# GiannisPikoulis/dsml-thesis

Hardware: AMD Instinct MI355X
Metric: DDIM denoise steps/sec (64×64×4 latent, 256² face) at 1/2/4/8 GPUs (higher is better)
Workload: dtype f32; 1 GPU; face_reenactment emotion-conditioned LDM (AffectNet config), DDIM-200 schedule, 16 samples/GPU, 64x64x4 latent, CFG off, eta 0, random-init weights; batch_per_gpu=16, global_batch=16, ddim_steps=200, hipgraph=True

## Files before the change

dsml_thesis_amd/csrc/igemm.hip:

```cpp
#include "ldmk_common.h"
#include "ldmk_split.h"
#include "ldmk_epilogue.h"
#include <stdlib.h>

#if defined(LDMK_IG_STAMPS) && (LDMK_IG_STAMPS == 1 || LDMK_IG_STAMPS == 3)
#define IG_T(i) do { const unsigned long long t_ = __builtin_amdgcn_s_memtime(); ig_acc[i] += t_ - ig_last; ig_last = t_; } while (0)
#elif defined(LDMK_IG_STAMPS)
#define IG_T(i) do { (void)ig_acc; (void)ig_last; } while (0)
#else
#define IG_T(i) do { } while (0)
#endif

namespace ldmk {

template <int TM, int TN, int LEAN>
__device__ __forceinline__ void ig_lean_epilogue(const ldmk_igemm_args& p, f32x16 (&acc)[TM][TN], const int rowbase, const int colbase, const int bz,
                                                 const int l31, const int half) {
  float* __restrict__ outp = p.out + (long long)bz * p.out_bstride;
  const float* __restrict__ resp = (LEAN == 2 || LEAN == 4) ? p.residual + (long long)bz * p.out_bstride : nullptr;
  const float alpha = p.alpha;
#pragma unroll
  for (int j = 0; j < TN; ++j) {
    const int col = colbase + j * 32 + l31;
    const float bv = p.bias ? p.bias[col] : 0.f;
// ... 1166 lines not shown
}

static int g_force_cfg = 0;
extern "C" void ldmk_igemm_force_config(int cfg) { g_force_cfg = cfg; }

extern "C" int ldmk_igemm_plan(const ldmk_igemm_args* args, int* tile_cfg, int* splitk) {
  if (!args || !tile_cfg || !splitk) return LDMK_EINVAL;
  ldmk::plan(*args, tile_cfg, splitk, args->splitk_ws ? args->splitk_ws_elems : 0);
  return LDMK_OK;
}

extern "C" long long ldmk_igemm_workspace_elems(const ldmk_igemm_args* args) {
  using namespace ldmk;
  LDMK_REQUIRE(args != nullptr, "ldmk_igemm_workspace_elems: null args");
  const ldmk_igemm_args& a = *args;
  LDMK_REQUIRE(a.M > 0 && a.N > 0 && a.K > 0, "ldmk_igemm_workspace_elems: empty problem M=%d N=%d K=%d", a.M, a.N, a.K);
  LDMK_REQUIRE(a.splitk >= 0 && a.splitk <= 64, "ldmk_igemm_workspace_elems: splitk=%d outside [0,64]", a.splitk);
  int cfg = a.tile_cfg, sk = a.splitk;
  if (sk == 0) {
    int c2 = 0;
    plan(a, &c2, &sk, 1LL << 50);
    if (cfg == 0) cfg = c2;
  }
  if (cfg > kNumCfg + kNumRCfg + kNumSCfg)
    return sk <= 1 || a.epi == LDMK_EPI_GEGLU ? 0 : (long long)(a.batch > 1 ? a.batch : 1) * sk * (long long)a.M * a.N;
  if (cfg > kNumCfg + kNumRCfg) {
    if (sk <= 1 || (a.epi == LDMK_EPI_GEGLU && !a.raw_slabs)) return 0;
    return (long long)sk * (long long)a.M * a.N;
  }
  if (cfg > kNumCfg || a.epi == LDMK_EPI_GEGLU || sk <= 1) return 0;
  return (long long)(a.batch > 1 ? a.batch : 1) * sk * (long long)a.M * a.N;
}

static int igemm_entry(const ldmk_igemm_args* args, void* stream, bool launch);
extern "C" int ldmk_igemm(const ldmk_igemm_args* args, void* stream) { return igemm_entry(args, stream, true); }
extern "C" int ldmk_igemm_check(const ldmk_igemm_args* args) { return igemm_entry(args, nullptr, false); }

static int igemm_entry(const ldmk_igemm_args* args, void* stream, bool launch) {
  LDMK_ENTER();
  using namespace ldmk;
  LDMK_REQUIRE(args != nullptr, "ldmk_igemm: null args");
  ldmk_igemm_args a = *args;
  LDMK_REQUIRE(a.M > 0 && a.N > 0 && a.K > 0, "ldmk_igemm: empty problem M=%d N=%d K=%d", a.M, a.N, a.K);
  LDMK_REQUIRE(a.c0 > 0 && a.c0 % 32 == 0 && a.c1 % 32 == 0, "ldmk_igemm: channel counts must be multiples of 32 (c0=%d c1=%d)", a.c0, a.c1);
  LDMK_REQUIRE((a.c1 == 0) == (a.a1 == nullptr), "ldmk_igemm: a1/c1 mismatch");
  const int taps = a.a_mode == LDMK_A_CONV3X3 ? 9 : 1;
  const int skip_k = a.skip_a0 ? a.skip_c0 + a.skip_c1 : 0;
  LDMK_REQUIRE(a.K == taps * (a.c0 + a.c1) + skip_k, "ldmk_igemm: K=%d != taps*(c0+c1)+skip=%d", a.K, taps * (a.c0 + a.c1) + skip_k);
  LDMK_REQUIRE(!a.skip_a0 || (a.a_mode == LDMK_A_CONV3X3 && a.skip_c0 > 0 && a.skip_c0 % 8 == 0 && a.skip_c1 % 8 == 0 &&
                              (a.skip_c1 == 0) == (a.skip_a1 == nullptr) && (a.tile_cfg > kNumCfg + kNumRCfg || a.tile_cfg == 0)),
               "ldmk_igemm: the fused skip connection needs a 3x3 convolution on a slab-GEMM tile, skip channels in multiples of 8");
  LDMK_REQUIRE(a.N % 4 == 0 && a.ldb % 4 == 0, "ldmk_igemm: N and ldb must be multiples of 4");
  LDMK_REQUIRE(a.rows_per_sample > 0, "ldmk_igemm: rows_per_sample");
  LDMK_REQUIRE((long long)a.M * a.ldc < (1LL << 31) && a.ldc > 0, "ldmk_igemm: output exceeds 2^31 elements per batch item (32-bit epilogue offsets)");
  const long long samples = ((long long)a.M + a.rows_per_sample - 1) / a.rows_per_sample;
  if (a.a_mode == LDMK_A_CONV3X3) {
    LDMK_REQUIRE(a.in_h > 0 && a.in_w > 0 && a.out_h > 0 && a.out_w > 0 && a.stride >= 1, "ldmk_igemm: conv geometry");
    LDMK_REQUIRE(a.rows_per_sample == a.out_h * a.out_w, "ldmk_igemm: rows_per_sample != out_h*out_w");
    LDMK_REQUIRE(a.batch <= 1, "ldmk_igemm: batched conv unsupported");
    LDMK_REQUIRE(samples * a.in_h * a.in_w * (a.c0 > a.c1 ? a.c0 : a.c1) < (1LL << 31),
                 "ldmk_igemm: conv input exceeds 2^31 elements (32-bit gather indices)");
  } else {
    LDMK_REQUIRE((long long)a.M * (a.c0 > a.c1 ? a.c0 : a.c1) < (1LL << 31), "ldmk_igemm: A exceeds 2^31 elements per batch item");
  }
  if (a.a_tf == LDMK_TF_AFFINE || a.a_tf == LDMK_TF_AFFINE_SILU) LDMK_REQUIRE(a.tf_coef, "ldmk_igemm: tf_coef missing");
  if (a.a_tf == LDMK_TF_LAYERNORM) {
    LDMK_REQUIRE(a.row_stats && a.ln_gamma && a.ln_beta && a.a_mode == LDMK_A_ROWS, "ldmk_igemm: layernorm prologue args");
  }
  if (a.a_tf == LDMK_TF_LAYERNORM_FOLDED)
    LDMK_REQUIRE(a.row_stats && a.ln_colsum && a.a_mode == LDMK_A_ROWS && !a.stats_out && a.batch <= 1,
                 "ldmk_igemm: folded layernorm needs row_stats, ln_colsum (ldmk_fold_layernorm), rows mode, no stats_out, no batching");
  LDMK_REQUIRE(a.a_tf >= LDMK_TF_NONE && a.a_tf <= LDMK_TF_LAYERNORM_FOLDED, "ldmk_igemm: a_tf=%d", a.a_tf);
  if (a.epi == LDMK_EPI_GEGLU) LDMK_REQUIRE(a.N % 64 == 0 && !a.residual && !a.batch_vec, "ldmk_igemm: GEGLU needs N%%64==0 and no residual");
  if (a.stats_out)
    LDMK_REQUIRE(a.M % 32 == 0 && a.rows_per_sample % 32 == 0 && a.epi == LDMK_EPI_NONE && a.batch <= 1,
                 "ldmk_igemm: stats_out needs M%%32==0, rows_per_sample%%32==0, no GEGLU, no batching");
  LDMK_REQUIRE(a.tile_cfg >= 0 && a.tile_cfg <= kNumCfg + kNumRCfg + kNumSCfg + kNumWCfg + kNumPCfg, "ldmk_igemm: tile_cfg=%d outside [0,%d]",
               a.tile_cfg, kNumCfg + kNumRCfg + kNumSCfg + kNumWCfg + kNumPCfg);
  LDMK_REQUIRE(a.splitk >= 0 && a.splitk <= 64, "ldmk_igemm: splitk=%d outside [0,64]", a.splitk);
  LDMK_REQUIRE(a.compute == LDMK_COMPUTE_F32 || a.compute == LDMK_COMPUTE_BF16 || a.compute == LDMK_COMPUTE_BF16X3 || a.compute == LDMK_COMPUTE_F16X2,
               "ldmk_igemm: compute=%d", a.compute);
  const bool ps_tile = a.tile_cfg > kNumCfg + kNumRCfg + kNumSCfg + kNumWCfg;
  LDMK_REQUIRE(!a.a_ps1 || (ps_tile && a.a_ps), "ldmk_igemm: a_ps1 (second A source) is read by the pre-split tiles only, next to a_ps");
  if (a.compute == LDMK_COMPUTE_BF16X3 && !ps_tile) {
    LDMK_REQUIRE(a.w_split && !a.b_trans && a.w_split_ld >= a.K && a.w_split_ld % 8 == 0,
                 "ldmk_igemm: LDMK_COMPUTE_BF16X3 needs w_split (ldmk_pack_wsplit), b_trans = 0, w_split_ld >= K and a multiple of 8");
    LDMK_REQUIRE(3LL * a.N * a.w_split_ld * 2 < (1LL << 32), "ldmk_igemm: w_split exceeds 4 GB per batch entry");
    LDMK_REQUIRE(igemm_fast_gather_ok(a), "ldmk_igemm: LDMK_COMPUTE_BF16X3 needs the fast gather (no zero-insertion, two-source "
                 "upsampling or operands beyond 4 GB)");
  }
  if (a.compute == LDMK_COMPUTE_F16X2) {
    LDMK_REQUIRE(a.tile_cfg <= kNumCfg || ps_tile, "ldmk_igemm: LDMK_COMPUTE_F16X2 runs on the LDS-tiled shapes (tile_cfg 0..6) and the pre-split "
                 "tiles (23..28, 31..33), not tile_cfg=%d", a.tile_cfg);
    LDMK_REQUIRE(!a.a_split && a.w_scale_exp >= -60 && a.w_scale_exp <= 60, "ldmk_igemm: LDMK_COMPUTE_F16X2: a_split is not taken; w_scale_exp=%d", a.w_scale_exp);
    if (!ps_tile) {
      LDMK_REQUIRE(a.w_split && !a.b_trans && a.w_split_ld >= a.K && a.w_split_ld % 8 == 0 && 2LL * a.N * a.w_split_ld * 2 < (1LL << 32),
                   "ldmk_igemm: LDMK_COMPUTE_F16X2 needs w_split (ldmk_pack_wsplit_h2), b_trans = 0, w_split_ld >= K and a multiple of 8, below 4 GB");
      LDMK_REQUIRE(a.range_flag != nullptr, "ldmk_igemm: LDMK_COMPUTE_F16X2 needs range_flag");
      LDMK_REQUIRE(igemm_fast_gather_ok(a), "ldmk_igemm: LDMK_COMPUTE_F16X2 needs the fast gather (no zero-insertion, two-source upsampling or "
                   "operands beyond 4 GB)");
    }
  }
  if (a.compute == LDMK_COMPUTE_BF16 && a.w_split)
    LDMK_REQUIRE(!a.b_trans && a.w_split_ld >= a.K && a.w_split_ld % 8 == 0 && (long long)a.N * a.w_split_ld * 2 < (1LL << 32) && a.batch <= 1,
                 "ldmk_igemm: LDMK_COMPUTE_BF16 with w_split (ldmk_pack_wbf16t) needs b_trans = 0, w_split_ld >= K and a multiple of 8, "
                 "no batching");
  if (a.a_split) {
    LDMK_REQUIRE(a.compute == LDMK_COMPUTE_BF16X3 && a.a_mode == LDMK_A_ROWS && a.c1 == 0 && a.batch <= 1 &&
                 (a.a_tf == LDMK_TF_NONE || a.a_tf == LDMK_TF_LAYERNORM_FOLDED) && a.tile_cfg <= kNumCfg,
                 "ldmk_igemm: a_split (pre-split A) needs LDMK_COMPUTE_BF16X3 on an LDS-tiled shape (tile_cfg 0..6), rows mode, one "
                 "source, no staging prologue, no batching");
    LDMK_REQUIRE(a.a_split_ld >= a.K && a.a_split_ld % 8 == 0 && 3LL * a.M * a.a_split_ld * 2 < (1LL << 32),
                 "ldmk_igemm: a_split_ld=%d must be >= K, a multiple of 8, and the three images below 4 GB", a.a_split_ld);
  }
  LDMK_REQUIRE(a.compute == LDMK_COMPUTE_F32 || a.tile_cfg <= kNumCfg || a.tile_cfg > kNumCfg + kNumRCfg + kNumSCfg,
               "ldmk_igemm: the row / slab GEMM tiles are fp32 only");
  if (a.alpha == 0.f) a.alpha = 1.f;
  if (a.compute == LDMK_COMPUTE_F16X2) a.alpha *= ldexpf(1.f, -(LDMK_F16X2_A_EXP + a.w_scale_exp));
  int cfg = 0, sk = 1;
  plan(a, &cfg, &sk, a.splitk_ws ? a.splitk_ws_elems : 0);
  if (a.tile_cfg > 0) cfg = a.tile_cfg;
  if (g_force_cfg > 0 && (g_force_cfg <= kNumCfg || !rgemm_unsupported(a, g_force_cfg - kNumCfg - 1))) cfg = g_force_cfg;
  LDMK_REQUIRE(!a.skip_a0 || cfg > kNumCfg + kNumRCfg, "ldmk_igemm: the fused skip connection runs on the slab GEMM only (tile_cfg 13..20)");
  if (cfg > kNumCfg + kNumRCfg + kNumSCfg + kNumWCfg) {
    const int pcfg = cfg - kNumCfg - kNumRCfg - kNumSCfg - kNumWCfg - 1;
    int psk = a.splitk > 0 ? a.splitk : 1;
    const char* why = igemm_ps_unsupported(a, pcfg, psk);
    LDMK_REQUIRE(why == nullptr, "ldmk_igemm: tile_cfg=%d splitk=%d (pre-split bf16x3 tile) cannot run this problem: %s", cfg, psk, why ? why : "");
    LDMK_REQUIRE(!a.raw_slabs || psk >= 2, "ldmk_igemm: raw_slabs needs a split-K plan");
    if (psk > 1) {
      const long long b = a.batch > 1 ? a.batch : 1;
      LDMK_REQUIRE_MEM(a.splitk_ws && b * psk * (long long)a.M * a.N <= a.splitk_ws_elems,
                       "ldmk_igemm: splitk=%d needs a workspace of %lld floats (ldmk_igemm_workspace_elems), %lld given", psk,
                       b * psk * (long long)a.M * a.N, a.splitk_ws ? a.splitk_ws_elems : 0LL);
    }
    if (!launch) return LDMK_OK;
    return igemm_ps_dispatch(a, pcfg, psk, a.splitk_ws, (hipStream_t)stream);
  }
  if (cfg > kNumCfg + kNumRCfg + kNumSCfg) {
    const int wcfg = cfg - kNumCfg - kNumRCfg - kNumSCfg - 1;
    int wsk = a.splitk > 0 ? a.splitk : 1;
    const char* why = igemm_ws_unsupported(a, wcfg, wsk);
    LDMK_REQUIRE(why == nullptr, "ldmk_igemm: tile_cfg=%d splitk=%d (warp-specialised bf16x3 tile) cannot run this problem: %s", cfg, wsk,
                 why ? why : "");
    LDMK_REQUIRE(!a.raw_slabs || wsk >= 2, "ldmk_igemm: raw_slabs needs a split-K plan");
    if (wsk > 1) {
      const long long b = a.batch > 1 ? a.batch : 1;
      LDMK_REQUIRE_MEM(a.splitk_ws && b * wsk * (long long)a.M * a.N <= a.splitk_ws_elems,
                       "ldmk_igemm: splitk=%d needs a workspace of %lld floats (ldmk_igemm_workspace_elems), %lld given", wsk,
                       b * wsk * (long long)a.M * a.N, a.splitk_ws ? a.splitk_ws_elems : 0LL);
    }
    if (!launch) return LDMK_OK;
    return igemm_ws_dispatch(a, wcfg, wsk, a.splitk_ws, (hipStream_t)stream);
  }
  if (cfg > kNumCfg + kNumRCfg) {
    const int scfg = cfg - kNumCfg - kNumRCfg - 1;
    int ssk = a.splitk > 0 ? a.splitk : 1;
    const char* why = sgemm_unsupported(a, scfg, ssk);
    LDMK_REQUIRE(why == nullptr, "ldmk_igemm: tile_cfg=%d splitk=%d (slab GEMM) cannot run this problem: %s", cfg, ssk, why ? why : "");
    if (ssk > 1)
      LDMK_REQUIRE_MEM(a.splitk_ws && ssk * (long long)a.M * a.N <= a.splitk_ws_elems,
                       "ldmk_igemm: splitk=%d needs a workspace of %lld floats (ldmk_igemm_workspace_elems), %lld given", ssk,
                       ssk * (long long)a.M * a.N, a.splitk_ws ? a.splitk_ws_elems : 0LL);
    if (!launch) return LDMK_OK;
    return sgemm_dispatch(a, scfg, ssk, a.splitk_ws, (hipStream_t)stream);
  }
// ... 28 lines not shown
```

dsml_thesis_amd/csrc/igemm_ps.hip:

```cpp
#include "ldmk_common.h"
#include "ldmk_split.h"
#include "ldmk_epilogue.h"
#include <stdlib.h>

namespace ldmk {

#ifdef LDMK_PS_PROBES
constexpr bool PS_PROBES = true;
#else
constexpr bool PS_PROBES = false;
#endif
static int ps_probe_bits() {
  if (!PS_PROBES) return 0;
  static const int dbg = [] {
    const char* d = getenv("LDMK_PS_DEBUG");
    const char* s = getenv("LDMK_PS_STAGGER");
    return (d ? atoi(d) : 0) | ((s ? atoi(s) : 0) << 8);
  }();
  return dbg;
}

constexpr unsigned PS_OOB = 0x80000000u;

__device__ __forceinline__ void ps_dma3(unsigned voff, const u32x4& rs, unsigned lds_dst) {
  unsigned keep;
  asm volatile("s_nop 4\n\ts_mov_b32 %0, m0\n\ts_mov_b32 m0, %3\n\ts_nop 0\n\t"
               "buffer_load_dwordx4 %1, %2, 0 offen lds\n\t"
               "buffer_load_dwordx4 %1, %2, 0 offen offset:1024 lds\n\t"
               "buffer_load_dwordx4 %1, %2, 0 offen offset:2048 lds\n\t"
               "s_mov_b32 m0, %0"
               : "=&s"(keep) : "v"(voff), "s"(rs), "s"(lds_dst) : "memory");
}

template <int PL>
__device__ __forceinline__ void ps_dma(unsigned voff, const u32x4& rs, unsigned lds_dst) {
  if constexpr (PL == 3) {
    ps_dma3(voff, rs, lds_dst);
  } else {
    unsigned keep;
    asm volatile("s_nop 4\n\ts_mov_b32 %0, m0\n\ts_mov_b32 m0, %3\n\ts_nop 0\n\t"
                 "buffer_load_dwordx4 %1, %2, 0 offen lds\n\t"
                 "buffer_load_dwordx4 %1, %2, 0 offen offset:1024 lds\n\t"
                 "s_mov_b32 m0, %0"
                 : "=&s"(keep) : "v"(voff), "s"(rs), "s"(lds_dst) : "memory");
  }
}

__device__ __attribute__((aligned(16))) const float kPsZeros[4] = {0.f, 0.f, 0.f, 0.f};

constexpr int PS_KV_TILE = 16 * 1024;
template <int TM, int TN, bool TR, int PL = 3, bool KV = false, int LEAN = 0>
__device__ __forceinline__ void ps_epilogue(const ldmk_igemm_args& p, f32x16 (&acc)[TM][TN], const int rowbase, const int colbase,
                                            const int splitk, const int ks, const int bz, float* __restrict__ ws, const int lane,
                                            float* __restrict__ kv_ts = nullptr) {
  const int l31 = lane & 31, half = lane >> 5;
  const float alpha = p.alpha;
  constexpr bool L_ANY = LEAN != 0, L_LNF = LEAN == 1, L_RS = LEAN == 2 || LEAN == 4, L_BV = LEAN == 4;
  const bool lnf = L_ANY ? L_LNF : p.a_tf == LDMK_TF_LAYERNORM_FOLDED;
  const float2* __restrict__ stats2 = reinterpret_cast<const float2*>(p.row_stats);

  if constexpr (TR) {
    if (splitk > 1) {
      float* slab = ws + ((long long)bz * splitk + ks) * p.M * p.N;
#pragma unroll
      for (int i = 0; i < TM; ++i) {
        const int row = rowbase + 32 * i + l31;
        if (row >= p.M) continue;
#pragma unroll
        for (int j = 0; j < TN; ++j)
#pragma unroll
          for (int q = 0; q < 4; ++q) {
            const int col = colbase + 32 * j + 8 * q + 4 * half;
            if (col < p.N)
              *reinterpret_cast<float4*>(slab + (long long)row * p.N + col) =
                  make_float4(acc[i][j][4 * q], acc[i][j][4 * q + 1], acc[i][j][4 * q + 2], acc[i][j][4 * q + 3]);
          }
      }
      return;
    }
    float* __restrict__ outp = p.out ? p.out + (long long)bz * p.out_bstride : nullptr;
    unsigned char* __restrict__ ops_ = reinterpret_cast<unsigned char*>(p.out_ps);
    const bool geglu = p.epi == LDMK_EPI_GEGLU;
    const int Kbo = p.ldc / 16;
    const float* __restrict__ csp = lnf ? p.ln_colsum : kPsZeros;
    const float* __restrict__ bip = p.bias ? p.bias : kPsZeros;
    const float* __restrict__ rsp = p.residual ? p.residual + (long long)bz * p.out_bstride : kPsZeros;
    const unsigned mcs = lnf ? ~0u : 0u, mbi = p.bias ? ~0u : 0u, mrs = p.residual ? ~0u : 0u, mbv = p.batch_vec ? ~0u : 0u;
    bool bad_ps = false;
#pragma unroll
    for (int i = 0; i < TM; ++i) {
      const int row = rowbase + 32 * i + l31;
      const bool rok = L_ANY || row < p.M;
      const int rr = rok ? row : p.M - 1;
      float mean = 0.f, rstd = 1.f;
      if (lnf) { const float2 st = stats2[rr]; mean = st.x; rstd = st.y; }
      const float* __restrict__ bvp = p.batch_vec ? p.batch_vec + (long long)(rr / p.rows_per_sample) * p.batch_vec_ld : kPsZeros;
      const unsigned rowoff = (unsigned)rr * (unsigned)p.ldc;
      const long long psrow = ((long long)((rowbase + 32 * i) >> 5) * Kbo) * (PL * 1024) + l31 * 16 + half * 8;
      constexpr int JS = (TN % 2 == 0) ? 2 : 1;
#pragma unroll
      for (int j = 0; j < TN; j += JS) {
#pragma unroll
        for (int jj = 0; jj < JS; ++jj) {
          if (geglu && jj == 1) break;
          const int jt = j + jj;
          const int ctile = colbase + 32 * jt;
          if (!L_ANY && ctile >= p.N) continue;
          const int otile = geglu ? (ctile >> 1) : ctile;
          float kvv[KV ? 16 : 1];
          const bool kv_tile = KV && ctile >= p.N / 3;
#pragma unroll
          for (int qh = 0; qh < 4; qh += 2) {
          float4 cs[4], bi[4], bv[4], rs[4], csg[4], big[4];
#pragma unroll
          for (int q = qh; q < qh + 2; ++q) {
            const unsigned c = (unsigned)(ctile + 8 * q + 4 * half), oc = (unsigned)(otile + 8 * q + 4 * half);
            if constexpr (!L_ANY || L_LNF) cs[q] = *reinterpret_cast<const float4*>(csp + (c & mcs));
            bi[q] = *reinterpret_cast<const float4*>(bip + (c & mbi));
            if constexpr (!L_ANY) {
              bv[q] = *reinterpret_cast<const float4*>(bvp + (oc & mbv));
              rs[q] = *reinterpret_cast<const float4*>(rsp + ((rowoff + oc) & mrs));
            } else {
              if constexpr (L_RS) rs[q] = *reinterpret_cast<const float4*>(rsp + (rowoff + oc));
              if constexpr (L_BV) bv[q] = *reinterpret_cast<const float4*>(bvp + oc);
            }
            if constexpr (TN % 2 == 0) {
              if (geglu) {
                if constexpr (!L_ANY || L_LNF) csg[q] = *reinterpret_cast<const float4*>(csp + ((c + 32) & mcs));
                big[q] = *reinterpret_cast<const float4*>(bip + ((c + 32) & mbi));
              }
            }
          }
#pragma unroll
          for (int q = qh; q < qh + 2; ++q) {
            float4 v = make_float4(acc[i][jt][4 * q] * alpha, acc[i][jt][4 * q + 1] * alpha, acc[i][jt][4 * q + 2] * alpha,
                                   acc[i][jt][4 * q + 3] * alpha);
            if constexpr (L_LNF) {
              v.x = lnf_bias(v.x, mean, cs[q].x, rstd, bi[q].x); v.y = lnf_bias(v.y, mean, cs[q].y, rstd, bi[q].y);
              v.z = lnf_bias(v.z, mean, cs[q].z, rstd, bi[q].z); v.w = lnf_bias(v.w, mean, cs[q].w, rstd, bi[q].w);
            } else if constexpr (L_ANY) {
            } else {
              if (lnf) {
                v.x = fmaf(-mean, cs[q].x, v.x) * rstd; v.y = fmaf(-mean, cs[q].y, v.y) * rstd;
                v.z = fmaf(-mean, cs[q].z, v.z) * rstd; v.w = fmaf(-mean, cs[q].w, v.w) * rstd;
              }
              v.x += bi[q].x; v.y += bi[q].y; v.z += bi[q].z; v.w += bi[q].w;
            }
            if constexpr (TN % 2 == 0) {
              if (geglu) {
                constexpr int TNm1 = TN - 1;
                const int jg = jt + 1 < TN ? jt + 1 : TNm1;
                float4 g = make_float4(acc[i][jg][4 * q] * alpha, acc[i][jg][4 * q + 1] * alpha, acc[i][jg][4 * q + 2] * alpha,
                                       acc[i][jg][4 * q + 3] * alpha);
                if constexpr (L_LNF) {
                  g.x = lnf_bias(g.x, mean, csg[q].x, rstd, big[q].x); g.y = lnf_bias(g.y, mean, csg[q].y, rstd, big[q].y);
                  g.z = lnf_bias(g.z, mean, csg[q].z, rstd, big[q].z); g.w = lnf_bias(g.w, mean, csg[q].w, rstd, big[q].w);
                } else {
                  if (lnf) {
                    g.x = fmaf(-mean, csg[q].x, g.x) * rstd; g.y = fmaf(-mean, csg[q].y, g.y) * rstd;
                    g.z = fmaf(-mean, csg[q].z, g.z) * rstd; g.w = fmaf(-mean, csg[q].w, g.w) * rstd;
                  }
                  g.x += big[q].x; g.y += big[q].y; g.z += big[q].z; g.w += big[q].w;
                }
                v.x *= gelu_erf_f(g.x); v.y *= gelu_erf_f(g.y); v.z *= gelu_erf_f(g.z); v.w *= gelu_erf_f(g.w);
              }
            }
            if constexpr (L_LNF) {
              v.x += 0.f; v.y += 0.f; v.z += 0.f; v.w += 0.f;
            } else if constexpr (L_ANY) {
              const float4 r4 = L_RS ? rs[q] : make_float4(0.f, 0.f, 0.f, 0.f), b4 = L_BV ? bv[q] : make_float4(0.f, 0.f, 0.f, 0.f);
              v.x = bias_res(v.x, bi[q].x, b4.x, r4.x); v.y = bias_res(v.y, bi[q].y, b4.y, r4.y);
              v.z = bias_res(v.z, bi[q].z, b4.z, r4.z); v.w = bias_res(v.w, bi[q].w, b4.w, r4.w);
            } else {
              v.x += bv[q].x; v.y += bv[q].y; v.z += bv[q].z; v.w += bv[q].w;
              v.x += rs[q].x; v.y += rs[q].y; v.z += rs[q].z; v.w += rs[q].w;
            }
            if constexpr (KV) {
              if (kv_tile) { kvv[4 * q] = v.x; kvv[4 * q + 1] = v.y; kvv[4 * q + 2] = v.z; kvv[4 * q + 3] = v.w; }
            }
            if (rok && !kv_tile) {
              const int oc = otile + 8 * q + 4 * half;
              if (outp) *reinterpret_cast<float4*>(outp + rowoff + oc) = v;
              if (ops_) {
                unsigned char* d = ops_ + psrow + (long long)((otile >> 4) + (q >> 1)) * (PL * 1024) + (q & 1) * 512;
                if constexpr (PL == 3) {
                  bf16x4 h, m, l;
                  split3(v, h, m, l);
                  *reinterpret_cast<bf16x4*>(d) = h;
                  *reinterpret_cast<bf16x4*>(d + 1024) = m;
                  *reinterpret_cast<bf16x4*>(d + 2048) = l;
                } else {
                  bad_ps |= h2_out_of_range(v);
                  f16x4 h, l;
                  split2h(scaled_sat(v), h, l);
                  *reinterpret_cast<f16x4*>(d) = h;
                  *reinterpret_cast<f16x4*>(d + 1024) = l;
                }
              }
            }
          }
          }
          if constexpr (KV) {
            if (kv_tile && (L_ANY || rowbase + 32 * i < p.M)) {
              const int Cq = p.N / 3;
              const int sec = ctile / Cq;
              const int hh = (ctile - sec * Cq) >> 5;
              const int r0 = rowbase + 32 * i;
              const int bsm = r0 / p.attn_tokens, key0 = r0 - bsm * p.attn_tokens;
              const int ntl = p.attn_tokens >> 6;
              unsigned char* dst = reinterpret_cast<unsigned char*>(p.attn_kv_out) +
                                   (((long long)bsm * (Cq >> 5) + hh) * ntl + (key0 >> 6)) * PS_KV_TILE + lane * 16;
              const int sub = (key0 >> 5) & 1;
              bool bad = false;
              if (sec == 1) {
#pragma unroll
                for (int t = 0; t < 2; ++t) {
                  float vals[8];
#pragma unroll
                  for (int e = 0; e < 4; ++e) {
                    const auto r = __builtin_amdgcn_permlane32_swap(__float_as_uint(kvv[8 * t + e]), __float_as_uint(kvv[8 * t + 4 + e]), false, false);
                    vals[e] = __uint_as_float(r[0]);
                    vals[4 + e] = __uint_as_float(r[1]);
                  }
                  const float4 v0 = make_float4(vals[0], vals[1], vals[2], vals[3]), v1 = make_float4(vals[4], vals[5], vals[6], vals[7]);
                  bad |= h2_out_of_range(v0) || h2_out_of_range(v1);
                  f16x4 h0, l0, h1, l1;
                  split2h(scaled_sat(v0), h0, l0);
                  split2h(scaled_sat(v1), h1, l1);
                  unsigned char* d = dst + (2 * sub + t) * 2048;
                  *reinterpret_cast<f16x8*>(d) = f16x8{h0[0], h0[1], h0[2], h0[3], h1[0], h1[1], h1[2], h1[3]};
                  *reinterpret_cast<f16x8*>(d + 1024) = f16x8{l0[0], l0[1], l0[2], l0[3], l1[0], l1[1], l1[2], l1[3]};
                }
              } else {
#pragma unroll
                for (int q = 0; q < 4; ++q)
#pragma unroll
                  for (int e = 0; e < 4; ++e) kv_ts[l31 * 33 + 8 * q + 4 * half + e] = kvv[4 * q + e];
                __builtin_amdgcn_s_waitcnt(0xC07F);
                __builtin_amdgcn_wave_barrier();
#pragma unroll
                for (int t = 0; t < 2; ++t) {
                  float vals[8];
#pragma unroll
                  for (int jx = 0; jx < 8; ++jx) vals[jx] = kv_ts[(16 * t + 4 * half + (jx & 3) + 8 * (jx >> 2)) * 33 + l31];
                  const float4 v0 = make_float4(vals[0], vals[1], vals[2], vals[3]), v1 = make_float4(vals[4], vals[5], vals[6], vals[7]);
                  bad |= h2_out_of_range(v0) || h2_out_of_range(v1);
                  f16x4 h0, l0, h1, l1;
                  split2h(scaled_sat(v0), h0, l0);
                  split2h(scaled_sat(v1), h1, l1);
                  unsigned char* d = dst + (4 + 2 * sub + t) * 2048;
                  *reinterpret_cast<f16x8*>(d) = f16x8{h0[0], h0[1], h0[2], h0[3], h1[0], h1[1], h1[2], h1[3]};
                  *reinterpret_cast<f16x8*>(d + 1024) = f16x8{l0[0], l0[1], l0[2], l0[3], l1[0], l1[1], l1[2], l1[3]};
                }
                __builtin_amdgcn_s_waitcnt(0xC07F);
                __builtin_amdgcn_wave_barrier();
              }
              if (bad) *p.range_flag = 1;
            }
          }
        }
      }
    }
    if (bad_ps) *p.range_flag = 1;
    return;
  } else {
    if (splitk > 1) {
      col_slab_store<TM, TN>(p, acc, rowbase, colbase, bz, l31, half, splitk, ks, ws);
      return;
    }
    if (p.epi == LDMK_EPI_GEGLU) {
      col_geglu<TM, TN>(p, acc, rowbase, colbase, bz, l31, half, lnf);
      return;
    }
    if constexpr (LEAN != 0) col_lean<TM, TN, LEAN>(p, acc, rowbase, colbase, bz, l31, half);
    else col_general<TM, TN>(p, acc, rowbase, colbase, bz, l31, half, lnf);
  }
}

template <bool TR>
__device__ __forceinline__ int ps_lean_form(const ldmk_igemm_args& p, const int splitk, const bool off, const int row_end, const int col_end) {
  if constexpr (!TR) {
    return col_lean_form(p, splitk, off, row_end, col_end);
  } else {
    if (off || splitk != 1 || row_end > p.M || col_end > p.N) return 0;
    if (p.batch_vec && p.rows_per_sample % 32 != 0) return 0;
    if (p.a_tf == LDMK_TF_LAYERNORM_FOLDED) return p.residual || p.batch_vec ? 0 : 1;
    if (p.epi == LDMK_EPI_GEGLU || (p.batch_vec && !p.residual)) return 0;
    return p.batch_vec ? 4 : (p.residual ? 2 : 3);
  }
}

template <int NWM, int NWN, int TM, int TN, int NS, bool TR, int PL = 3, bool KV = false>
__global__ __launch_bounds__(64 * NWM * NWN, 2) void igemm_ps_kernel(const ldmk_igemm_args p, const int splitk, float* __restrict__ ws, const int dbg_arg, const int nfast) {
  const int dbg = PS_PROBES ? dbg_arg : 0;
  constexpr int NW = NWM * NWN;
  constexpr int BM = 32 * TM * NWM, BN = 32 * TN * NWN;
  constexpr int FA = BM / 32, FB = BN / 32, U = FA + FB;
  constexpr int UHI = (U + NW - 1) / NW, ULO = U / NW;
  constexpr int UB = PL * 1024;
  constexpr int STAGE = U * UB;
  static_assert(PL * UHI * (NS - 1) <= 63, "vmcnt is a 6-bit counter");
  extern __shared__ __attribute__((aligned(1024))) unsigned char smem_ps[];

  const int tid = threadIdx.x, lane = tid & 63, wave = __builtin_amdgcn_readfirstlane(tid >> 6);
  const int l31 = lane & 31, half = lane >> 5;
  const int wm = wave / NWN, wn = wave - wm * NWN;

  const int tiles_m = (p.M + BM - 1) / BM;
  const int tiles_n = (p.N + BN - 1) / BN;
  const int bid = xcd_remap(blockIdx.x, tiles_m * tiles_n);
  const int m0 = (nfast & 1) ? (bid / tiles_n) * BM : (bid % tiles_m) * BM;
  const int n0 = (nfast & 1) ? (bid % tiles_n) * BN : (bid / tiles_m) * BN;
  const int ks = blockIdx.y, bz = blockIdx.z;

  const int nkc = p.K / 32;
  const int it_per = (nkc + splitk - 1) / splitk;
  const int it_begin = ks * it_per;
  const int it_end = min(nkc, it_begin + it_per);
  const int n16 = it_end > it_begin ? 2 * (it_end - it_begin) : 0;
  const int Kb = p.K / 16;
  const int Mb = (p.M + 31) / 32, Nb = p.N / 32;

  const int Ka0 = p.a_ps1 ? p.a_ps_k0 / 16 : Kb, Ka1 = Kb - Ka0;
  const u32x4 rs_a = buffer_rsrc(reinterpret_cast<const unsigned char*>(p.a_ps) + (long long)bz * p.a_ps_bstride, (dbg & 1) ? 0u : (unsigned)Mb * (unsigned)Ka0 * (unsigned)UB);
  const u32x4 rs_a1 = buffer_rsrc(p.a_ps1 ? p.a_ps1 : p.a_ps, (dbg & 1) ? 0u : (unsigned)Mb * (unsigned)Ka1 * (unsigned)UB);
  const u32x4 rs_b = buffer_rsrc(reinterpret_cast<const unsigned char*>(p.w_ps) + (long long)bz * p.w_ps_bstride, (dbg & 1) ? 0u : (unsigned)Nb * (unsigned)Kb * (unsigned)UB);
  unsigned ubase[UHI], ubase1[UHI];
#pragma unroll
  for (int i = 0; i < UHI; ++i) {
    const int u = wave + NW * i;
    const int blk = u < FA ? m0 / 32 + u : n0 / 32 + (u - FA);
    const bool ok = u < U && (u < FA ? blk < Mb : blk < Nb);
    ubase[i] = ok ? (unsigned)blk * (unsigned)(u < FA ? Ka0 : Kb) * (unsigned)UB + (unsigned)(2 * it_begin) * (unsigned)UB : PS_OOB;
    ubase1[i] = (unsigned)blk * (unsigned)Ka1 * (unsigned)UB + (unsigned)(2 * it_begin - Ka0) * (unsigned)UB;
  }
  const unsigned lane16 = lane * 16;
  const unsigned lds0 = (unsigned)(size_t)smem_ps;
  auto issue = [&](int s) {
    const unsigned buf = lds0 + (unsigned)(s % NS) * STAGE;
    const bool live = s < n16;
    const bool src1 = 2 * it_begin + s >= Ka0;
    const u32x4 rs_as = src1 ? rs_a1 : rs_a;
#pragma unroll
    for (int i = 0; i < UHI; ++i) {
      const int u = wave + NW * i;
      if (u < U && !(dbg & 2)) {
        const unsigned off = (live && ubase[i] != PS_OOB) ? ((u < FA && src1) ? ubase1[i] : ubase[i]) + (unsigned)s * (unsigned)UB : PS_OOB;
        ps_dma<PL>(lane16 + off, u < FA ? rs_as : rs_b, buf + (unsigned)u * (unsigned)UB);
      }
    }
  };
  const bool hi_wave = wave + NW * (UHI - 1) < U;

  f32x16 acc[TM][TN];
#pragma unroll
  for (int i = 0; i < TM; ++i)
#pragma unroll
    for (int j = 0; j < TN; ++j)
#pragma unroll
      for (int r = 0; r < 16; ++r) acc[i][j][r] = 0.f;

  if ((dbg >> 8) != 0) {
    const unsigned slot = __builtin_amdgcn_s_getreg(6148);
    if (slot & 1) {
      const int n = (dbg >> 8) * n16;
      for (int i = 0; i < n; i += 64) __builtin_amdgcn_s_sleep(64);
    }
  }
#pragma unroll
  for (int s = 0; s < NS - 1; ++s) issue(s);
  for (int it = 0; it < n16; ++it) {
    if (hi_wave) wait_vm<PL * UHI * (NS - 2)>(); else wait_vm<PL * ULO * (NS - 2)>();
    asm volatile("s_barrier" ::: "memory");
    issue(it + NS - 1);
    const unsigned char* sb = smem_ps + (it % NS) * STAGE + lane16;
    bf16x8 a8[PL][TM];
#pragma unroll
    for (int g = 0; g < PL; ++g)
#pragma unroll
      for (int i = 0; i < TM; ++i) a8[g][i] = *reinterpret_cast<const bf16x8*>(sb + ((wm * TM + i) * PL + g) * 1024);
#pragma unroll
    for (int j = 0; j < TN; ++j) {
      bf16x8 b8[PL];
#pragma unroll
      for (int g = 0; g < PL; ++g) b8[g] = *reinterpret_cast<const bf16x8*>(sb + ((FA + wn * TN + j) * PL + g) * 1024);
      if (dbg & 4) {
#pragma unroll
        for (int i = 0; i < TM; ++i)
#pragma unroll
          for (int g = 0; g < PL; ++g) asm volatile("" :: "v"(a8[g][i]), "v"(b8[g]));
        continue;
      }
#pragma unroll
      for (int i = 0; i < TM; ++i) {
        if constexpr (PL == 2) {
          const f16x8 ah = __builtin_bit_cast(f16x8, a8[0][i]), al = __builtin_bit_cast(f16x8, a8[1][i]);
          const f16x8 bh = __builtin_bit_cast(f16x8, b8[0]), bl = __builtin_bit_cast(f16x8, b8[1]);
          if constexpr (TR) {
            acc[i][j] = __builtin_amdgcn_mfma_f32_32x32x16_f16(bh, al, acc[i][j], 0, 0, 0);
            acc[i][j] = __builtin_amdgcn_mfma_f32_32x32x16_f16(bl, ah, acc[i][j], 0, 0, 0);
            acc[i][j] = __builtin_amdgcn_mfma_f32_32x32x16_f16(bh, ah, acc[i][j], 0, 0, 0);
          } else {
            acc[i][j] = __builtin_amdgcn_mfma_f32_32x32x16_f16(al, bh, acc[i][j], 0, 0, 0);
            acc[i][j] = __builtin_amdgcn_mfma_f32_32x32x16_f16(ah, bl, acc[i][j], 0, 0, 0);
            acc[i][j] = __builtin_amdgcn_mfma_f32_32x32x16_f16(ah, bh, acc[i][j], 0, 0, 0);
          }
        } else if constexpr (TR) {
          acc[i][j] = __builtin_amdgcn_mfma_f32_32x32x16_bf16(b8[0], a8[2][i], acc[i][j], 0, 0, 0);
          acc[i][j] = __builtin_amdgcn_mfma_f32_32x32x16_bf16(b8[2], a8[0][i], acc[i][j], 0, 0, 0);
          acc[i][j] = __builtin_amdgcn_mfma_f32_32x32x16_bf16(b8[1], a8[1][i], acc[i][j], 0, 0, 0);
          acc[i][j] = __builtin_amdgcn_mfma_f32_32x32x16_bf16(b8[0], a8[1][i], acc[i][j], 0, 0, 0);
          acc[i][j] = __builtin_amdgcn_mfma_f32_32x32x16_bf16(b8[1], a8[0][i], acc[i][j], 0, 0, 0);
          acc[i][j] = __builtin_amdgcn_mfma_f32_32x32x16_bf16(b8[0], a8[0][i], acc[i][j], 0, 0, 0);
        } else {
          acc[i][j] = __builtin_amdgcn_mfma_f32_32x32x16_bf16(a8[2][i], b8[0], acc[i][j], 0, 0, 0);
          acc[i][j] = __builtin_amdgcn_mfma_f32_32x32x16_bf16(a8[0][i], b8[2], acc[i][j], 0, 0, 0);
          acc[i][j] = __builtin_amdgcn_mfma_f32_32x32x16_bf16(a8[1][i], b8[1], acc[i][j], 0, 0, 0);
          acc[i][j] = __builtin_amdgcn_mfma_f32_32x32x16_bf16(a8[1][i], b8[0], acc[i][j], 0, 0, 0);
          acc[i][j] = __builtin_amdgcn_mfma_f32_32x32x16_bf16(a8[0][i], b8[1], acc[i][j], 0, 0, 0);
          acc[i][j] = __builtin_amdgcn_mfma_f32_32x32x16_bf16(a8[0][i], b8[0], acc[i][j], 0, 0, 0);
        }
      }
    }
  }
  wait_vm<0>();
  if (dbg & 16) {
    float keep = 0.f;
#pragma unroll
    for (int i = 0; i < TM; ++i)
#pragma unroll
      for (int j = 0; j < TN; ++j)
#pragma unroll
        for (int r = 0; r < 16; ++r) keep += acc[i][j][r];
    if (keep == 12345.678f && ws) ws[0] = keep;
    return;
  }
  const int lean = ps_lean_form<TR>(p, splitk, (nfast & 2) != 0, m0 + (wm + 1) * 32 * TM, n0 + (wn + 1) * 32 * TN);
  if constexpr (KV) {
    __syncthreads();
    if (lean == 1)
      ps_epilogue<TM, TN, TR, PL, true, TR ? 1 : 0>(p, acc, m0 + wm * 32 * TM, n0 + wn * 32 * TN, splitk, ks, bz, ws, lane,
                                                    reinterpret_cast<float*>(smem_ps) + wave * (32 * 33));
    else
      ps_epilogue<TM, TN, TR, PL, true>(p, acc, m0 + wm * 32 * TM, n0 + wn * 32 * TN, splitk, ks, bz, ws, lane,
                                         reinterpret_cast<float*>(smem_ps) + wave * (32 * 33));
  } else {
    if (lean == 1) ps_epilogue<TM, TN, TR, PL, false, 1>(p, acc, m0 + wm * 32 * TM, n0 + wn * 32 * TN, splitk, ks, bz, ws, lane);
    else if (lean == 2) ps_epilogue<TM, TN, TR, PL, false, 2>(p, acc, m0 + wm * 32 * TM, n0 + wn * 32 * TN, splitk, ks, bz, ws, lane);
    else if (lean == 3) ps_epilogue<TM, TN, TR, PL, false, 3>(p, acc, m0 + wm * 32 * TM, n0 + wn * 32 * TN, splitk, ks, bz, ws, lane);
    else if (lean == 4) ps_epilogue<TM, TN, TR, PL, false, 4>(p, acc, m0 + wm * 32 * TM, n0 + wn * 32 * TN, splitk, ks, bz, ws, lane);
    else ps_epilogue<TM, TN, TR, PL>(p, acc, m0 + wm * 32 * TM, n0 + wn * 32 * TN, splitk, ks, bz, ws, lane);
  }
}

template <int TM, int TN, int NS, bool TR>
__global__ __launch_bounds__(512) void igemm_pw_kernel(const ldmk_igemm_args p, const int splitk, float* __restrict__ ws, const int dbg_arg) {
  const int dbg = PS_PROBES ? dbg_arg : 0;
  constexpr int BM = 128 * TM, BN = 32 * TN;
  constexpr int FA = BM / 32, FB = TN, U = FA + FB;
  constexpr int UHI = (U + 3) / 4, ULO = U / 4;
  constexpr int STAGE = U * 3072;
  static_assert(NS >= 3 && 3 * UHI * (NS - 2) <= 63, "ring depth / vmcnt range");
  extern __shared__ __attribute__((aligned(1024))) unsigned char smem_ps[];

  const int tid = threadIdx.x, lane = tid & 63, wave = __builtin_amdgcn_readfirstlane(tid >> 6);
  const int tiles_m = (p.M + BM - 1) / BM;
  const int tiles_n = (p.N + BN - 1) / BN;
  const int bid = xcd_remap(blockIdx.x, tiles_m * tiles_n);
  const int m0 = (bid % tiles_m) * BM;
  const int n0 = (bid / tiles_m) * BN;
  const int ks = blockIdx.y, bz = blockIdx.z;
  const int nkc = p.K / 32;
  const int it_per = (nkc + splitk - 1) / splitk;
  const int it_begin = ks * it_per;
  const int it_end = min(nkc, it_begin + it_per);
  const int n16 = it_end > it_begin ? 2 * (it_end - it_begin) : 0;
  const unsigned lane16 = lane * 16;

  if (wave >= 4) {
    const int pw = wave - 4;
    const int Kb = p.K / 16;
    const int Mb = (p.M + 31) / 32, Nb = p.N / 32;
    const u32x4 rs_a = buffer_rsrc(reinterpret_cast<const unsigned char*>(p.a_ps) + (long long)bz * p.a_ps_bstride, (dbg & 1) ? 0u : (unsigned)Mb * (unsigned)Kb * 3072u);
    const u32x4 rs_b = buffer_rsrc(reinterpret_cast<const unsigned char*>(p.w_ps) + (long long)bz * p.w_ps_bstride, (dbg & 1) ? 0u : (unsigned)Nb * (unsigned)Kb * 3072u);
    unsigned ubase[UHI];
#pragma unroll
    for (int i = 0; i < UHI; ++i) {
      const int u = pw + 4 * i;
      const int blk = u < FA ? m0 / 32 + u : n0 / 32 + (u - FA);
      const bool ok = u < U && (u < FA ? blk < Mb : blk < Nb);
      ubase[i] = ok ? (unsigned)blk * (unsigned)Kb * 3072u + (unsigned)(2 * it_begin) * 3072u : PS_OOB;
    }
    const unsigned lds0 = (unsigned)(size_t)smem_ps;
    auto issue = [&](int s) {
      const unsigned buf = lds0 + (unsigned)(s % NS) * STAGE;
      const bool live = s < n16;
#pragma unroll
      for (int i = 0; i < UHI; ++i) {
        const int u = pw + 4 * i;
        if (u < U && !(dbg & 2)) {
          const unsigned off = (live && ubase[i] != PS_OOB) ? ubase[i] + (unsigned)s * 3072u : PS_OOB;
          ps_dma3(lane16 + off, u < FA ? rs_a : rs_b, buf + (unsigned)u * 3072u);
        }
      }
    };
    const bool hi_wave = pw + 4 * (UHI - 1) < U;
    unsigned long long t_acc[3] = {0, 0, 0}, t_last = __builtin_amdgcn_s_memtime();
    const unsigned long long t_begin = t_last;
#define PW_T(i) do { if (dbg & 8) { const unsigned long long t_ = __builtin_amdgcn_s_memtime(); t_acc[i] += t_ - t_last; t_last = t_; } } while (0)
#pragma unroll
    for (int s = 0; s < NS - 1; ++s) issue(s);
    PW_T(0);
    if (hi_wave) wait_vm<3 * UHI * (NS - 2)>(); else wait_vm<3 * ULO * (NS - 2)>();
    PW_T(1);
    asm volatile("s_barrier" ::: "memory");
    PW_T(2);
    for (int it = 0; it < n16; ++it) {
      if (hi_wave) wait_vm<3 * UHI * (NS - 3)>(); else wait_vm<3 * ULO * (NS - 3)>();
      PW_T(1);
      asm volatile("s_barrier" ::: "memory");
      PW_T(2);
      issue(it + NS - 1);
      PW_T(0);
    }
    wait_vm<0>();
    if ((dbg & 8) && lane == 0 && p.splitk_counters) {
      unsigned long long* d = reinterpret_cast<unsigned long long*>(p.splitk_counters) + ((long long)blockIdx.x * 8 + wave) * 4;
      d[0] = t_acc[0]; d[1] = t_acc[1]; d[2] = t_acc[2]; d[3] = __builtin_amdgcn_s_memtime() - t_begin;
    }
    return;
// ... 120 lines not shown
    split3(make_float4(v[0], v[1], v[2], v[3]), h0, m0, l0);
    split3(make_float4(v[4], v[5], v[6], v[7]), h1, m1, l1);
    *reinterpret_cast<bf16x8*>(d) = bf16x8{h0[0], h0[1], h0[2], h0[3], h1[0], h1[1], h1[2], h1[3]};
    *reinterpret_cast<bf16x8*>(d + 1024) = bf16x8{m0[0], m0[1], m0[2], m0[3], m1[0], m1[1], m1[2], m1[3]};
    *reinterpret_cast<bf16x8*>(d + 2048) = bf16x8{l0[0], l0[1], l0[2], l0[3], l1[0], l1[1], l1[2], l1[3]};
  }
}

template <int KCH, int PL = 3>
__global__ __launch_bounds__(256) void ln_stats_ps_kernel(const float* __restrict__ x, int rows, int K, float eps, float* __restrict__ stats,
                                                          unsigned char* __restrict__ dst, float guard, int* __restrict__ flag,
                                                          int* __restrict__ range_flag) {
  const int rb = blockIdx.x;
  const int r = threadIdx.x >> 3, o = threadIdx.x & 7;
  const int row = rb * 32 + r;
  const bool rok = row < rows;
  const float* px = x + (long long)(rok ? row : 0) * K;
  float4 v[KCH][2];
  float s = 0.f;
#pragma unroll
  for (int c = 0; c < KCH; ++c) {
    const int k0 = c * 64 + o * 8;
    if (rok && k0 < K) {
      v[c][0] = *reinterpret_cast<const float4*>(px + k0);
      v[c][1] = *reinterpret_cast<const float4*>(px + k0 + 4);
    } else {
      v[c][0] = v[c][1] = make_float4(0.f, 0.f, 0.f, 0.f);
    }
    s += ((v[c][0].x + v[c][0].y) + (v[c][0].z + v[c][0].w)) + ((v[c][1].x + v[c][1].y) + (v[c][1].z + v[c][1].w));
  }
#pragma unroll
  for (int d = 4; d > 0; d >>= 1) s += __shfl_xor(s, d, 64);
  const float mean = s / (float)K;
  float q = 0.f;
#pragma unroll
  for (int c = 0; c < KCH; ++c) {
    if (c * 64 + o * 8 < K) {
#pragma unroll
      for (int e = 0; e < 2; ++e) {
        const float a = v[c][e].x - mean, b = v[c][e].y - mean, cc = v[c][e].z - mean, d = v[c][e].w - mean;
        q = fmaf(a, a, q); q = fmaf(b, b, q); q = fmaf(cc, cc, q); q = fmaf(d, d, q);
      }
    }
  }
#pragma unroll
  for (int d = 4; d > 0; d >>= 1) q += __shfl_xor(q, d, 64);
  if (rok && o == 0) {
    const float rstd = 1.0f / sqrtf(q / (float)K + eps);
    stats[2 * (long long)row] = mean;
    stats[2 * (long long)row + 1] = rstd;
    if (flag && !(fabsf(mean) * rstd <= guard)) *flag = 1;
  }
#pragma unroll
  for (int c = 0; c < KCH; ++c) {
    const int k0 = c * 64 + o * 8;
    if (k0 < K) {
      unsigned char* d = dst + ((long long)rb * (K / 16) + (k0 >> 4)) * (PL * 1024) + ((o & 1) * 32 + r) * 16;
      if constexpr (PL == 2) {
        if (h2_out_of_range(v[c][0]) || h2_out_of_range(v[c][1])) *range_flag = 1;
        f16x4 h0, l0, h1, l1;
        split2h(scaled_sat(v[c][0]), h0, l0);
        split2h(scaled_sat(v[c][1]), h1, l1);
        *reinterpret_cast<f16x8*>(d) = f16x8{h0[0], h0[1], h0[2], h0[3], h1[0], h1[1], h1[2], h1[3]};
        *reinterpret_cast<f16x8*>(d + 1024) = f16x8{l0[0], l0[1], l0[2], l0[3], l1[0], l1[1], l1[2], l1[3]};
      } else {
        bf16x4 h0, m0, l0, h1, m1, l1;
        split3(v[c][0], h0, m0, l0);
        split3(v[c][1], h1, m1, l1);
        *reinterpret_cast<bf16x8*>(d) = bf16x8{h0[0], h0[1], h0[2], h0[3], h1[0], h1[1], h1[2], h1[3]};
        *reinterpret_cast<bf16x8*>(d + 1024) = bf16x8{m0[0], m0[1], m0[2], m0[3], m1[0], m1[1], m1[2], m1[3]};
        *reinterpret_cast<bf16x8*>(d + 2048) = bf16x8{l0[0], l0[1], l0[2], l0[3], l1[0], l1[1], l1[2], l1[3]};
      }
    }
  }
}

int launch_splitk_reduce(const ldmk_igemm_args& a, int splitk, float* ws, hipStream_t st);

struct PsCfg { int bm, bn; bool even_tn; };
static const PsCfg kPsCfg[] = {{256, 160, false}, {256, 320, false}, {256, 256, true}, {128, 320, false}, {128, 160, false}, {128, 256, true},
                               {256, 160, false}, {256, 128, true},
                               {256, 160, false}, {256, 128, true}, {128, 256, true}};

template <int NWM, int NWN, int TM, int TN, int NS, bool TR, int PL = 3, bool KV = false>
static int ps_launch(const ldmk_igemm_args& a, int splitk, float* ws, hipStream_t st) {
  constexpr int BM = 32 * TM * NWM, BN = 32 * TN * NWN;
  constexpr size_t lds = (size_t)NS * (BM / 32 + BN / 32) * PL * 1024;
  static_assert(lds <= 160 * 1024, "LDS ring exceeds 160 KiB");
  static bool attr = false;
  if (!attr) {
    (void)hipFuncSetAttribute(reinterpret_cast<const void*>(igemm_ps_kernel<NWM, NWN, TM, TN, NS, TR, PL, KV>),
                              hipFuncAttributeMaxDynamicSharedMemorySize, (int)lds);
    attr = true;
  }
  const int tiles = ((a.M + BM - 1) / BM) * ((a.N + BN - 1) / BN);
  const int dbg = ps_probe_bits();
  static_assert(!KV || (size_t)NWM * NWN * 32 * 33 * 4 <= lds, "V^T transpose scratch fits the ring");
  const int nfast_env = switch_value(SW_PS_NFAST);
  const int lean_env = switch_value(SW_PS_LEAN);
  const int nfast = (nfast_env && (a.N + BN - 1) / BN > 1 && (a.M + BM - 1) / BM >= 8 ? 1 : 0) | (lean_env ? 0 : 2);
  hipLaunchKernelGGL((igemm_ps_kernel<NWM, NWN, TM, TN, NS, TR, PL, KV>), dim3(tiles, splitk, a.batch > 1 ? a.batch : 1), dim3(64 * NWM * NWN), lds,
                     st, a, splitk, ws, dbg, nfast);
  if (splitk > 1 && !a.raw_slabs) return launch_splitk_reduce(a, splitk, ws, st);
  return check_launch("ldmk_igemm(ps)");
}

template <int TM, int TN, int NS, bool TR>
static int pw_launch(const ldmk_igemm_args& a, int splitk, float* ws, hipStream_t st) {
  constexpr int BM = 128 * TM, BN = 32 * TN;
  constexpr size_t lds = (size_t)NS * (BM / 32 + TN) * 3072;
  static_assert(lds <= 160 * 1024, "LDS ring exceeds 160 KiB");
  static bool attr = false;
  if (!attr) {
    (void)hipFuncSetAttribute(reinterpret_cast<const void*>(igemm_pw_kernel<TM, TN, NS, TR>), hipFuncAttributeMaxDynamicSharedMemorySize, (int)lds);
    attr = true;
  }
  const int tiles = ((a.M + BM - 1) / BM) * ((a.N + BN - 1) / BN);
  const int dbg = ps_probe_bits() & 0xff;
  hipLaunchKernelGGL((igemm_pw_kernel<TM, TN, NS, TR>), dim3(tiles, splitk, a.batch > 1 ? a.batch : 1), dim3(512), lds, st, a, splitk, ws, dbg);
  if (splitk > 1 && !a.raw_slabs) return launch_splitk_reduce(a, splitk, ws, st);
  return check_launch("ldmk_igemm(pw)");
}

template <int NWM, int NWN, int TM, int TN, bool TR>
__global__ __launch_bounds__(64 * NWM * NWN, 2) void igemm_psc_kernel(const ldmk_igemm_args p, const int splitk, float* __restrict__ ws, const int nfast) {
  constexpr int PL = 2, NS = 3;
  constexpr int NW = NWM * NWN;
  constexpr int BM = 32 * TM * NWM, BN = 32 * TN * NWN;
  constexpr int FA = BM / 32, FB = BN / 32, U = FA + FB;
  constexpr int UHI = (U + NW - 1) / NW, ULO = U / NW;
  constexpr int AI = (FA + NW - 1) / NW;
  constexpr int UB = PL * 1024;
  constexpr int STAGE = U * UB;
  static_assert(18 % NS == 0 && PL * UHI * (NS - 1) <= 63, "ring / vmcnt");
  extern __shared__ __attribute__((aligned(1024))) unsigned char smem_ps[];

  const int tid = threadIdx.x, lane = tid & 63, wave = __builtin_amdgcn_readfirstlane(tid >> 6);
  const int l31 = lane & 31, half = lane >> 5;
  const int wm = wave / NWN, wn = wave - wm * NWN;
  const int tiles_m = (p.M + BM - 1) / BM;
  const int tiles_n = (p.N + BN - 1) / BN;
  const int bid = xcd_remap(blockIdx.x, tiles_m * tiles_n);
  const int m0 = (nfast & 1) ? (bid / tiles_n) * BM : (bid % tiles_m) * BM;
  const int n0 = (nfast & 1) ? (bid % tiles_n) * BN : (bid / tiles_m) * BN;
  const int ks = blockIdx.y;

  const int C = p.c0;
  const int nc32 = C / 32;
  const int c_per = (nc32 + splitk - 1) / splitk;
  const int c_begin = ks * c_per;
  const int c_end = min(nc32, c_begin + c_per);
  const int Kb_in = C / 16, Kb_w = p.K / 16;
  const int Nb = p.N / 32;
  const long long samples = ((long long)p.M + p.rows_per_sample - 1) / p.rows_per_sample;
  const unsigned Mb_in = (unsigned)((samples * p.in_h * p.in_w + 31) / 32);
  const u32x4 rs_a = buffer_rsrc(p.a_ps, Mb_in * (unsigned)Kb_in * (unsigned)UB);
  const u32x4 rs_b = buffer_rsrc(p.w_ps, (unsigned)Nb * (unsigned)Kb_w * (unsigned)UB);

  unsigned toff[AI][9];
#pragma unroll
  for (int i = 0; i < AI; ++i) {
    const int u = wave + NW * i;
    const int row = m0 + 32 * u + l31;
    const bool rok = u < FA && row < p.M;
    const int rr = rok ? row : 0;
    const int n = rr / p.rows_per_sample, rem = rr - n * p.rows_per_sample;
    const int oy = rem / p.out_w, ox = rem - oy * p.out_w;
#pragma unroll
    for (int t = 0; t < 9; ++t) {
      const int iy = oy * p.stride + t / 3 - p.pad_lo, ix = ox * p.stride + t % 3 - p.pad_lo;
      const bool ok = rok && iy >= 0 && iy < p.in_h && ix >= 0 && ix < p.in_w;
      const unsigned q = (unsigned)((n * p.in_h + iy) * p.in_w + ix);
      toff[i][t] = ok ? (q >> 5) * (unsigned)Kb_in * (unsigned)UB + ((unsigned)half * 32u + (q & 31u)) * 16u : PS_OOB;
    }
  }
  unsigned ubase[UHI];
#pragma unroll
  for (int i = 0; i < UHI; ++i) {
    const int u = wave + NW * i;
    const int blk = n0 / 32 + (u - FA);
    ubase[i] = (u >= FA && u < U && blk < Nb) ? (unsigned)blk * (unsigned)Kb_w * (unsigned)UB + (unsigned)(18 * c_begin) * (unsigned)UB : PS_OOB;
  }
  const unsigned lane16 = lane * 16;
  const unsigned lds0 = (unsigned)(size_t)smem_ps;
// ... 80 lines not shown
  const int k0 = kc * 64 + o * 8;
  if (k0 >= C) return;
  float4 v0 = make_float4(0.f, 0.f, 0.f, 0.f), v1 = v0;
  if (row < rows) {
    const float* src = k0 < c0 ? x0 + row * c0 + k0 : x1 + row * c1 + (k0 - c0);
    const float4 a = *reinterpret_cast<const float4*>(src), b = *reinterpret_cast<const float4*>(src + 4);
    const float* cf = coef + ((row / hw) * 2) * C + k0;
    const float4 s0 = *reinterpret_cast<const float4*>(cf), s1 = *reinterpret_cast<const float4*>(cf + 4);
    const float4 h0 = *reinterpret_cast<const float4*>(cf + C), h1 = *reinterpret_cast<const float4*>(cf + C + 4);
    v0 = make_float4(fmaf(a.x, s0.x, h0.x), fmaf(a.y, s0.y, h0.y), fmaf(a.z, s0.z, h0.z), fmaf(a.w, s0.w, h0.w));
    v1 = make_float4(fmaf(b.x, s1.x, h1.x), fmaf(b.y, s1.y, h1.y), fmaf(b.z, s1.z, h1.z), fmaf(b.w, s1.w, h1.w));
    if (silu) {
      v0 = make_float4(silu_f(v0.x), silu_f(v0.y), silu_f(v0.z), silu_f(v0.w));
      v1 = make_float4(silu_f(v1.x), silu_f(v1.y), silu_f(v1.z), silu_f(v1.w));
    }
    if (h2_out_of_range(v0) || h2_out_of_range(v1)) *range_flag = 1;
  }
  unsigned char* d = dst + ((long long)rb * (C / 16) + (k0 >> 4)) * 2048 + ((o & 1) * 32 + r) * 16;
  f16x4 a0, l0, a1, l1;
  split2h(scaled_sat(v0), a0, l0);
  split2h(scaled_sat(v1), a1, l1);
  *reinterpret_cast<f16x8*>(d) = f16x8{a0[0], a0[1], a0[2], a0[3], a1[0], a1[1], a1[2], a1[3]};
  *reinterpret_cast<f16x8*>(d + 1024) = f16x8{l0[0], l0[1], l0[2], l0[3], l1[0], l1[1], l1[2], l1[3]};
}

template <int NWM, int NWN, int TM, int TN, bool TR>
static int psc_launch(const ldmk_igemm_args& a, int splitk, float* ws, hipStream_t st) {
  constexpr int BM = 32 * TM * NWM, BN = 32 * TN * NWN;
  constexpr size_t lds = (size_t)3 * (BM / 32 + BN / 32) * 2048;
  static_assert(lds <= 160 * 1024, "LDS ring exceeds 160 KiB");
  static bool attr = false;
  if (!attr) {
    (void)hipFuncSetAttribute(reinterpret_cast<const void*>(igemm_psc_kernel<NWM, NWN, TM, TN, TR>), hipFuncAttributeMaxDynamicSharedMemorySize, (int)lds);
    attr = true;
  }
  const int tiles = ((a.M + BM - 1) / BM) * ((a.N + BN - 1) / BN);
  const int nfast_env = switch_value(SW_PS_NFAST);
  const int lean_env = switch_value(SW_PS_LEAN);
  const int nfast = (nfast_env && (a.N + BN - 1) / BN > 1 && (a.M + BM - 1) / BM >= 8 ? 1 : 0) | (lean_env ? 0 : 2);
  hipLaunchKernelGGL((igemm_psc_kernel<NWM, NWN, TM, TN, TR>), dim3(tiles, splitk, 1), dim3(64 * NWM * NWN), lds, st, a, splitk, ws, nfast);
  if (splitk > 1 && !a.raw_slabs) return launch_splitk_reduce(a, splitk, ws, st);
  return check_launch("ldmk_igemm(ps, conv)");
}

const char* igemm_ps_unsupported(const ldmk_igemm_args& a, int pcfg, int splitk) {
  if (a.compute != LDMK_COMPUTE_BF16X3 && a.compute != LDMK_COMPUTE_F16X2) return "the pre-split tiles run the bf16x3 and the f16x2 arithmetic (compute)";
  const int pl = a.compute == LDMK_COMPUTE_F16X2 ? 2 : 3;
  if (pl == 2 && (pcfg == 6 || pcfg == 7)) return "the warp-specialised pre-split tiles (29 / 30) exist in the bf16x3 arithmetic only";
  if (pl == 2 && a.out_ps && !a.range_flag) return "out_ps in the f16x2 arithmetic needs range_flag";
  if (!a.a_ps || !a.w_ps) return "a_ps / w_ps (operands in the PS layout: ldmk_pack_ps, ldmk_ln_stats_ps, out_ps of a producer GEMM)";
  if (a.a_mode == LDMK_A_CONV3X3) {
    if (pl != 2) return "the conv-mode pre-split tile runs the f16x2 arithmetic only";
    if (pcfg != 0 && pcfg != 1 && pcfg != 3 && pcfg != 4) return "conv mode: tile_cfg 23 / 24 / 26 / 27";
    if (a.c1 || a.a1 || a.upsample || a.a_tf != LDMK_TF_NONE || a.out_ps || a.batch > 1 || a.epi != LDMK_EPI_NONE || a.attn_kv_out)
      return "conv mode: one pre-normalised source (ldmk_gn_apply_ps_h2), no upsampling / prologue / out_ps / batching / GEGLU";
    if (a.c0 % 32) return "conv mode: C_in must be a multiple of 32";
    if ((a.c0 / 32) % splitk) return "conv mode: splitk must divide C_in / 32 (K is split on 32-channel chunk boundaries)";
    const long long smp = ((long long)a.M + a.rows_per_sample - 1) / a.rows_per_sample;
    if (((smp * a.in_h * a.in_w + 31) / 32) * (a.c0 / 16) * 2048 >= (1LL << 31)) return "conv mode: input of 2 GiB or more";
  } else if (a.a_mode != LDMK_A_ROWS) {
    return "rows mode or 3x3 convolution";
  }
  if (a.b_trans || a.upsample || a.skip_a0 || (a.splitk_counters && !(ps_probe_bits() & 8))) return "b_trans / upsample / fused skip / in-launch combine";
  if (a.a_tf != LDMK_TF_NONE && a.a_tf != LDMK_TF_LAYERNORM_FOLDED) return "no staging prologue: a_ps is what gets multiplied";
  if (a.K % 32 || a.N % 32) return "K and N must be multiples of 32";
  if (a.a_ps1) {
    if (a.a_mode != LDMK_A_ROWS || pcfg == 6 || pcfg == 7) return "a_ps1: rows mode on tile_cfg 23..28 / 31..33 (not the conv-mode or warp-specialised tiles)";
    if (a.batch > 1 || a.attn_kv_out || a.a_tf != LDMK_TF_NONE || a.epi == LDMK_EPI_GEGLU)
      return "a_ps1: no batching, no fused QKV tiles, no folded LayerNorm, no GEGLU";
    if (a.a_ps_k0 <= 0 || a.a_ps_k0 >= a.K || a.a_ps_k0 % 32) return "a_ps1: a_ps_k0 and K - a_ps_k0 must be positive multiples of 32";
  }
  const long long kb = a.K / 16;
  if ((a.a_mode == LDMK_A_ROWS && (long long)((a.M + 31) / 32) * kb * pl * 1024 >= (1LL << 31)) || (long long)(a.N / 32) * kb * pl * 1024 >= (1LL << 31))
    return "an operand of 2 GiB or more";
  if (a.epi == LDMK_EPI_GEGLU && (!kPsCfg[pcfg].even_tn || splitk > 1)) return "GEGLU needs a tile of (value, gate) pairs (256x256, 128x256) and no split-K";
  if (splitk > a.K / 32) return "more K slices than 32-deep chunks";
  if (a.out_ps) {
    if (splitk > 1 || a.batch > 1 || a.stats_out) return "out_ps: no split-K, no batching, no GroupNorm records (transposed epilogue)";
    if (a.ldc % 16) return "out_ps: ldc (the PS output's column count) must be a multiple of 16";
  } else if (!a.out && splitk <= 1) {
    return "no output";
  }
  if (a.stats_out && !a.out) return "stats_out needs out";
  if (a.attn_kv_out) {
    if (pl != 2 || (pcfg != 0 && pcfg != 4)) return "attn_kv_out: the F16X2 arithmetic on tile_cfg 23 / 27";
    if (a.stats_out || splitk > 1 || a.batch > 1 || a.epi != LDMK_EPI_NONE || a.out_ps || !a.out || !a.range_flag)
      return "attn_kv_out: the fused QKV projection (no split-K / batching / GEGLU / records / out_ps; out and range_flag required)";
    if (a.attn_heads <= 0 || a.N != 3 * 32 * a.attn_heads) return "attn_kv_out: N must be 3 x 32 x attn_heads ([q | k | v] of d_head 32)";
    if (a.attn_tokens <= 0 || a.attn_tokens % 64 || a.M % a.attn_tokens) return "attn_kv_out: attn_tokens a multiple of 64 that divides M";
  }
  return nullptr;
}

int igemm_ps_dispatch(const ldmk_igemm_args& a, int pcfg, int splitk, float* ws, hipStream_t st) {
  const bool tr = !a.stats_out;
  if (a.a_mode == LDMK_A_CONV3X3) {
    switch (pcfg) {
      case 0: return tr ? psc_launch<8, 1, 1, 5, true>(a, splitk, ws, st) : psc_launch<8, 1, 1, 5, false>(a, splitk, ws, st);
      case 1: return tr ? psc_launch<4, 2, 2, 5, true>(a, splitk, ws, st) : psc_launch<4, 2, 2, 5, false>(a, splitk, ws, st);
      case 3: return tr ? psc_launch<4, 2, 1, 5, true>(a, splitk, ws, st) : psc_launch<4, 2, 1, 5, false>(a, splitk, ws, st);
      default: return tr ? psc_launch<4, 1, 1, 5, true>(a, splitk, ws, st) : psc_launch<4, 1, 1, 5, false>(a, splitk, ws, st);
    }
  }
  if (a.compute == LDMK_COMPUTE_F16X2 && a.attn_kv_out)
    return pcfg == 0 ? ps_launch<8, 1, 1, 5, 3, true, 2, true>(a, splitk, ws, st) : ps_launch<4, 1, 1, 5, 3, true, 2, true>(a, splitk, ws, st);
  if (a.compute == LDMK_COMPUTE_F16X2) {
    switch (pcfg) {
      case 0: return tr ? ps_launch<8, 1, 1, 5, 3, true, 2>(a, splitk, ws, st) : ps_launch<8, 1, 1, 5, 3, false, 2>(a, splitk, ws, st);
      case 1: return tr ? ps_launch<4, 2, 2, 5, 3, true, 2>(a, splitk, ws, st) : ps_launch<4, 2, 2, 5, 3, false, 2>(a, splitk, ws, st);
      case 2: return tr ? ps_launch<4, 2, 2, 4, 3, true, 2>(a, splitk, ws, st) : ps_launch<4, 2, 2, 4, 3, false, 2>(a, splitk, ws, st);
      case 3: return tr ? ps_launch<4, 2, 1, 5, 3, true, 2>(a, splitk, ws, st) : ps_launch<4, 2, 1, 5, 3, false, 2>(a, splitk, ws, st);
      case 4: return tr ? ps_launch<4, 1, 1, 5, 3, true, 2>(a, splitk, ws, st) : ps_launch<4, 1, 1, 5, 3, false, 2>(a, splitk, ws, st);
      case 8: return tr ? ps_launch<4, 1, 2, 5, 3, true, 2>(a, splitk, ws, st) : ps_launch<4, 1, 2, 5, 3, false, 2>(a, splitk, ws, st);
      case 9: return tr ? ps_launch<4, 1, 2, 4, 3, true, 2>(a, splitk, ws, st) : ps_launch<4, 1, 2, 4, 3, false, 2>(a, splitk, ws, st);
      case 10: return tr ? ps_launch<2, 2, 2, 4, 3, true, 2>(a, splitk, ws, st) : ps_launch<2, 2, 2, 4, 3, false, 2>(a, splitk, ws, st);
      default: return tr ? ps_launch<4, 2, 1, 4, 3, true, 2>(a, splitk, ws, st) : ps_launch<4, 2, 1, 4, 3, false, 2>(a, splitk, ws, st);
    }
  }
  switch (pcfg) {
    case 0: return tr ? ps_launch<8, 1, 1, 5, 3, true>(a, splitk, ws, st) : ps_launch<8, 1, 1, 5, 3, false>(a, splitk, ws, st);
    case 1: return tr ? ps_launch<4, 2, 2, 5, 2, true>(a, splitk, ws, st) : ps_launch<4, 2, 2, 5, 2, false>(a, splitk, ws, st);
    case 2: return tr ? ps_launch<4, 2, 2, 4, 3, true>(a, splitk, ws, st) : ps_launch<4, 2, 2, 4, 3, false>(a, splitk, ws, st);
    case 3: return tr ? ps_launch<4, 2, 1, 5, 3, true>(a, splitk, ws, st) : ps_launch<4, 2, 1, 5, 3, false>(a, splitk, ws, st);
    case 4: return tr ? ps_launch<4, 1, 1, 5, 2, true>(a, splitk, ws, st) : ps_launch<4, 1, 1, 5, 2, false>(a, splitk, ws, st);
    case 6: return tr ? pw_launch<2, 5, 4, true>(a, splitk, ws, st) : pw_launch<2, 5, 4, false>(a, splitk, ws, st);
    case 7: return tr ? pw_launch<2, 4, 4, true>(a, splitk, ws, st) : pw_launch<2, 4, 4, false>(a, splitk, ws, st);
    case 8: return tr ? ps_launch<4, 1, 2, 5, 2, true>(a, splitk, ws, st) : ps_launch<4, 1, 2, 5, 2, false>(a, splitk, ws, st);
    case 9: return tr ? ps_launch<4, 1, 2, 4, 2, true>(a, splitk, ws, st) : ps_launch<4, 1, 2, 4, 2, false>(a, splitk, ws, st);
    case 10: return tr ? ps_launch<2, 2, 2, 4, 2, true>(a, splitk, ws, st) : ps_launch<2, 2, 2, 4, 2, false>(a, splitk, ws, st);
    default: return tr ? ps_launch<4, 2, 1, 4, 3, true>(a, splitk, ws, st) : ps_launch<4, 2, 1, 4, 3, false>(a, splitk, ws, st);
  }
}

}

extern "C" long long ldmk_ps_bytes(int rows, int k) {
  if (rows <= 0 || k <= 0 || k % 16) return -1;
  return (long long)((rows + 31) / 32) * (k / 16) * 3072;
}

extern "C" long long ldmk_ps_bytes_h2(int rows, int k) {
  if (rows <= 0 || k <= 0 || k % 16) return -1;
  return (long long)((rows + 31) / 32) * (k / 16) * 2048;
}

extern "C" int ldmk_pack_ps(const float* src, int rows, int k, long long row_stride, long long k_stride, int batch, long long src_bstride,
                            void* dst, void* stream) {
  LDMK_ENTER();
  using namespace ldmk;
  LDMK_REQUIRE(src && dst && rows > 0 && k > 0 && batch >= 1, "ldmk_pack_ps: bad args");
  LDMK_REQUIRE(k % 16 == 0, "ldmk_pack_ps: k=%d must be a multiple of 16", k);
  LDMK_REQUIRE(k_stride != 1 || (row_stride % 4 == 0 && (reinterpret_cast<uintptr_t>(src) & 15) == 0 && src_bstride % 4 == 0),
               "ldmk_pack_ps: row-major sources are read as float4 (16-byte aligned rows)");
  const long long bytes = ldmk_ps_bytes(rows, k);
  hipLaunchKernelGGL(pack_ps_kernel<3>, dim3((rows + 31) / 32, (k + 63) / 64, batch), dim3(256), 0, (hipStream_t)stream, src, rows, k, row_stride,
                     k_stride, src_bstride, reinterpret_cast<unsigned char*>(dst), bytes, 1.0f, (int*)nullptr);
  return check_launch("ldmk_pack_ps");
}

extern "C" int ldmk_pack_ps_h2(const float* src, int rows, int k, long long row_stride, long long k_stride, int batch, long long src_bstride,
                               int scale_exp, int* range_flag, void* dst, void* stream) {
  LDMK_ENTER();
  using namespace ldmk;
  LDMK_REQUIRE(src && dst && rows > 0 && k > 0 && batch >= 1, "ldmk_pack_ps_h2: bad args");
  LDMK_REQUIRE(k % 16 == 0, "ldmk_pack_ps_h2: k=%d must be a multiple of 16", k);
  LDMK_REQUIRE(k_stride != 1 || (row_stride % 4 == 0 && (reinterpret_cast<uintptr_t>(src) & 15) == 0 && src_bstride % 4 == 0),
               "ldmk_pack_ps_h2: row-major sources are read as float4 (16-byte aligned rows)");
  LDMK_REQUIRE(scale_exp >= -60 && scale_exp <= 60, "ldmk_pack_ps_h2: scale_exp=%d outside [-60, 60]", scale_exp);
  LDMK_REQUIRE(!range_flag || scale_exp == LDMK_F16X2_A_EXP, "ldmk_pack_ps_h2: range_flag is the activations' check: scale_exp must be %d", LDMK_F16X2_A_EXP);
  const long long bytes = ldmk_ps_bytes_h2(rows, k);
  hipLaunchKernelGGL(pack_ps_kernel<2>, dim3((rows + 31) / 32, (k + 63) / 64, batch), dim3(256), 0, (hipStream_t)stream, src, rows, k, row_stride,
                     k_stride, src_bstride, reinterpret_cast<unsigned char*>(dst), bytes, ldexpf(1.f, scale_exp), range_flag);
  return check_launch("ldmk_pack_ps_h2");
}

extern "C" int ldmk_ln_stats_ps(const float* x, int rows, int c, float eps, float* stats, void* dst, float guard, int* flag, void* stream) {
  LDMK_ENTER();
  using namespace ldmk;
  LDMK_REQUIRE(x && stats && dst && rows > 0 && c > 0, "ldmk_ln_stats_ps: bad args");
  LDMK_REQUIRE(c % 16 == 0 && c <= 1280, "ldmk_ln_stats_ps: C=%d must be a multiple of 16, at most 1280", c);
  LDMK_REQUIRE(!flag || guard > 0.f, "ldmk_ln_stats_ps: guard=%g must be positive", (double)guard);
  const dim3 grid((rows + 31) / 32);
  unsigned char* d = reinterpret_cast<unsigned char*>(dst);
  hipStream_t st = (hipStream_t)stream;
// ... 39 lines not shown
```

dsml_thesis_amd/lib.py:

```python
import ctypes as C
import os

from . import switches

_HERE = os.path.dirname(os.path.abspath(__file__))
LIB_PATH = switches.get("LDMK_LIBRARY") or os.path.join(_HERE, "libldmk.so")

A_ROWS, A_CONV3X3 = 0, 1
TF_NONE, TF_AFFINE, TF_AFFINE_SILU, TF_LAYERNORM, TF_LAYERNORM_FOLDED = 0, 1, 2, 3, 4
EPI_NONE, EPI_GEGLU = 0, 1
COMPUTE_F32, COMPUTE_BF16, COMPUTE_BF16X3, COMPUTE_F16X2 = 0, 1, 2, 3
POST_NONE, POST_GROUPNORM, POST_LAYERNORM = 0, 1, 2
PLMS_MULTISTEP, PLMS_PREDICTOR, PLMS_CORRECTOR = 0, 1, 2

_fp = C.c_void_p


class IgemmArgs(C.Structure):
    _fields_ = [
        ("M", C.c_int), ("N", C.c_int), ("K", C.c_int),
        ("a0", _fp), ("a1", _fp), ("c0", C.c_int), ("c1", C.c_int),
        ("a_mode", C.c_int), ("in_h", C.c_int), ("in_w", C.c_int), ("out_h", C.c_int), ("out_w", C.c_int),
        ("stride", C.c_int), ("pad_lo", C.c_int), ("upsample", C.c_int),
        ("a_tf", C.c_int), ("tf_coef", _fp), ("row_stats", _fp), ("ln_gamma", _fp), ("ln_beta", _fp),
        ("rows_per_sample", C.c_int),
        ("w", _fp), ("b_trans", C.c_int), ("ldb", C.c_int),
        ("bias", _fp), ("batch_vec", _fp), ("batch_vec_ld", C.c_int),
        ("residual", _fp), ("epi", C.c_int),
        ("out", _fp), ("ldc", C.c_int), ("batch", C.c_int),
        ("a_bstride", C.c_longlong), ("w_bstride", C.c_longlong), ("out_bstride", C.c_longlong),
        ("alpha", C.c_float), ("tile_cfg", C.c_int), ("splitk", C.c_int),
        ("splitk_ws", _fp), ("splitk_ws_elems", C.c_longlong), ("stats_out", _fp), ("compute", C.c_int), ("splitk_counters", _fp), ("splitk_counters_len", C.c_int),
        ("w_frag", _fp),
        ("ln_colsum", _fp),
        ("raw_slabs", C.c_int),
        ("skip_a0", _fp), ("skip_a1", _fp), ("skip_c0", C.c_int), ("skip_c1", C.c_int),
        ("w_split", _fp), ("w_split_ld", C.c_int), ("w_split_bstride", C.c_longlong),
        ("a_split", _fp), ("a_split_ld", C.c_int),
        ("a_ps", _fp), ("a_ps_bstride", C.c_longlong), ("w_ps", _fp), ("w_ps_bstride", C.c_longlong), ("out_ps", _fp),
        ("w_scale_exp", C.c_int), ("range_flag", _fp),
        ("attn_kv_out", _fp), ("attn_tokens", C.c_int), ("attn_heads", C.c_int),
        ("a_ps1", _fp), ("a_ps_k0", C.c_int),
    ]


class PostArgs(C.Structure):
    _fields_ = [
        ("src", _fp), ("nslab", C.c_int), ("slab_stride", C.c_longlong), ("M", C.c_int), ("N", C.c_int),
        ("rows_per_sample", C.c_int), ("alpha", C.c_float), ("bias", _fp), ("batch_vec", _fp), ("batch_vec_ld", C.c_int),
        ("residual", _fp), ("ldr", C.c_int), ("geglu", C.c_int), ("raw_out", _fp), ("ld_raw", C.c_int), ("norm", C.c_int),
        ("x1", _fp), ("c1", C.c_int), ("groups", C.c_int), ("eps", C.c_float), ("gamma", _fp), ("beta", _fp),
        ("silu", C.c_int), ("norm_out", _fp), ("ld_norm", C.c_int), ("gn_cache_floats", C.c_int),
        ("gn_scratch", _fp), ("gn_scratch_elems", C.c_longlong),
    ]


class WgradArgs(C.Structure):
    _fields_ = [
        ("R", C.c_int), ("Kw", C.c_int), ("N", C.c_int), ("a", _fp), ("c", C.c_int), ("lda", C.c_int),
        ("a_mode", C.c_int), ("in_h", C.c_int), ("in_w", C.c_int), ("out_h", C.c_int), ("out_w", C.c_int),
        ("stride", C.c_int), ("pad_lo", C.c_int), ("upsample", C.c_int),
        ("dy", _fp), ("ldy", C.c_int), ("dw", _fp), ("ldw", C.c_int), ("accumulate", C.c_int), ("alpha", C.c_float),
        ("batch", C.c_int), ("a_bstride", C.c_longlong), ("dy_bstride", C.c_longlong), ("dw_bstride", C.c_longlong),
        ("splitr", C.c_int), ("ws", _fp), ("ws_elems", C.c_longlong), ("dbias", _fp), ("compute", C.c_int),
    ]


_SIGS = {
    "ldmk_version": (C.c_int, []),
    "ldmk_last_error": (C.c_char_p, []),
    "ldmk_init": (C.c_int, [C.c_int]),
    "ldmk_switch_value": (C.c_int, [C.c_char_p]),
    "ldmk_switch_override": (C.c_int, [C.c_char_p, C.c_int]),
    "ldmk_igemm": (C.c_int, [C.POINTER(IgemmArgs), _fp]),
    "ldmk_igemm_workspace_elems": (C.c_longlong, [C.POINTER(IgemmArgs)]),
    "ldmk_igemm_check": (C.c_int, [C.POINTER(IgemmArgs)]),
    "ldmk_igemm_plan": (C.c_int, [C.POINTER(IgemmArgs), C.POINTER(C.c_int), C.POINTER(C.c_int)]),
    "ldmk_igemm_force_config": (None, [C.c_int]),
    "ldmk_wfrag_elems": (C.c_longlong, [C.c_int, C.c_int]),
    "ldmk_pack_wfrag": (C.c_int, [_fp, C.c_int, C.c_int, C.c_int, _fp, _fp]),
    "ldmk_pack_wsplit": (C.c_int, [_fp, C.c_int, C.c_int, C.c_int, C.c_int, C.c_longlong, _fp, C.c_int, _fp]),
    "ldmk_pack_wsplit_h2": (C.c_int, [_fp, C.c_int, C.c_int, C.c_int, C.c_int, C.c_longlong, C.c_int, _fp, C.c_int, _fp]),
    "ldmk_pack_wbf16t": (C.c_int, [_fp, C.c_int, C.c_int, C.c_int, _fp, C.c_int, _fp]),
    "ldmk_winograd_tiles": (C.c_longlong, [C.c_int, C.c_int, C.c_int]),
    "ldmk_winograd_input": (C.c_int, [_fp, C.c_int, _fp, C.c_int, _fp, C.c_int, C.c_int, C.c_int, C.c_int, _fp, _fp]),
    "ldmk_winograd_input_ps": (C.c_int, [_fp, C.c_int, _fp, C.c_int, _fp, C.c_int, C.c_int, C.c_int, C.c_int, _fp, _fp]),
    "ldmk_winograd_output": (C.c_int, [_fp, _fp, _fp, C.c_int, _fp, _fp, _fp, C.c_int, C.c_int, C.c_int, C.c_int, _fp]),
    "ldmk_upconv_gather": (C.c_int, [_fp, C.c_int, C.c_int, C.c_int, C.c_int, _fp, _fp]),
    "ldmk_upconv_gather_ps": (C.c_int, [_fp, C.c_int, C.c_int, C.c_int, C.c_int, _fp, _fp]),
    "ldmk_upconv_gather_ps_h2": (C.c_int, [_fp, C.c_int, C.c_int, C.c_int, C.c_int, _fp, _fp, _fp]),
    "ldmk_winograd_input_ps_h2": (C.c_int, [_fp, C.c_int, _fp, C.c_int, _fp, C.c_int, C.c_int, C.c_int, C.c_int, _fp, _fp, _fp]),
    "ldmk_winograd_input_ps_v1": (C.c_int, [_fp, C.c_int, _fp, C.c_int, _fp, C.c_int, C.c_int, C.c_int, C.c_int, _fp, _fp]),
    "ldmk_winograd_input_ps_h2_v1": (C.c_int, [_fp, C.c_int, _fp, C.c_int, _fp, C.c_int, C.c_int, C.c_int, C.c_int, _fp, _fp, _fp]),
    "ldmk_winograd_output_v1": (C.c_int, [_fp, _fp, _fp, C.c_int, _fp, _fp, _fp, C.c_int, C.c_int, C.c_int, C.c_int, _fp]),
    "ldmk_winograd_input_ps_route": (C.c_int, [C.c_int, C.c_int, C.c_int, C.c_int, C.c_int]),
    "ldmk_winograd_output_route": (C.c_int, [C.c_int, C.c_int, C.c_int, C.c_int, C.c_int]),
    "ldmk_upconv_scatter": (C.c_int, [_fp, _fp, _fp, _fp, C.c_int, C.c_int, C.c_int, C.c_int, _fp]),
    "ldmk_fold_layernorm": (C.c_int, [_fp, C.c_int, C.c_int, C.c_int, _fp, _fp, _fp, _fp, _fp, _fp, _fp]),
    "ldmk_attn_force_qt": (None, [C.c_int]),
    "ldmk_gn_chunks": (C.c_int, [C.c_int]),
    "ldmk_gn_partial": (C.c_int, [_fp, C.c_int, C.c_int, C.c_int, _fp, _fp]),
    "ldmk_gn_finalize": (C.c_int, [_fp, C.c_int, _fp, C.c_int, C.c_int, C.c_int, C.c_int, C.c_float, _fp, _fp, _fp, _fp]),
    "ldmk_gn_coef": (C.c_int, [_fp, C.c_int, _fp, C.c_int, C.c_int, C.c_int, C.c_int, C.c_float, _fp, _fp, _fp, _fp, _fp]),
    "ldmk_ln_stats": (C.c_int, [_fp, C.c_int, C.c_int, C.c_float, _fp, _fp]),
    "ldmk_ln_stats_guard": (C.c_int, [_fp, C.c_int, C.c_int, C.c_float, _fp, C.c_float, _fp, _fp]),
    "ldmk_ps_bytes": (C.c_longlong, [C.c_int, C.c_int]),
    "ldmk_pack_ps": (C.c_int, [_fp, C.c_int, C.c_int, C.c_longlong, C.c_longlong, C.c_int, C.c_longlong, _fp, _fp]),
    "ldmk_ps_bytes_h2": (C.c_longlong, [C.c_int, C.c_int]),
    "ldmk_pack_ps_h2": (C.c_int, [_fp, C.c_int, C.c_int, C.c_longlong, C.c_longlong, C.c_int, C.c_longlong, C.c_int, _fp, _fp, _fp]),
    "ldmk_ln_stats_ps_h2": (C.c_int, [_fp, C.c_int, C.c_int, C.c_float, _fp, _fp, C.c_float, _fp, _fp, _fp]),
    "ldmk_ln_stats_ps": (C.c_int, [_fp, C.c_int, C.c_int, C.c_float, _fp, _fp, C.c_float, _fp, _fp]),
    "ldmk_ln_stats_split": (C.c_int, [_fp, C.c_int, C.c_int, C.c_float, _fp, _fp, C.c_int, _fp]),
    "ldmk_gn_apply": (C.c_int, [_fp, C.c_int, _fp, C.c_int, _fp, _fp, C.c_int, C.c_int, C.c_int, _fp]),
    "ldmk_gn_coef_film": (C.c_int, [_fp, _fp, C.c_int, C.c_int, C.c_int, _fp]),
    "ldmk_gn_apply_ps_h2": (C.c_int, [_fp, C.c_int, _fp, C.c_int, _fp, _fp, C.c_int, C.c_int, C.c_int, _fp, _fp]),
    "ldmk_post": (C.c_int, [C.POINTER(PostArgs), _fp]),
    "ldmk_post_scratch_elems": (C.c_longlong, [C.POINTER(PostArgs)]),
    "ldmk_attn_self": (C.c_int, [_fp, _fp, C.c_int, C.c_int, C.c_int, C.c_float, _fp]),
    "ldmk_attn_self_x3": (C.c_int, [_fp, _fp, C.c_int, C.c_int, C.c_int, C.c_float, _fp]),
    "ldmk_attn_kv_split_bytes": (C.c_longlong, [C.c_int, C.c_int, C.c_int]),
    "ldmk_attn_self_x3p": (C.c_int, [_fp, _fp, _fp, C.c_int, C.c_int, C.c_int, C.c_float, _fp]),
    "ldmk_attn_self_x3p_ps": (C.c_int, [_fp, _fp, _fp, _fp, C.c_int, C.c_int, C.c_int, C.c_float, _fp]),
    "ldmk_attn_kv_split_h2_bytes": (C.c_longlong, [C.c_int, C.c_int, C.c_int]),
    "ldmk_attn_self_h2": (C.c_int, [_fp, _fp, _fp, _fp, C.c_int, C.c_int, C.c_int, C.c_float, _fp]),
    "ldmk_attn_self_h2_ps": (C.c_int, [_fp, _fp, _fp, _fp, _fp, C.c_int, C.c_int, C.c_int, C.c_float, _fp]),
# ... 145 lines not shown
```

dsml_thesis_amd/ops.py:

```python
import ctypes as C
import math
import weakref
from typing import NamedTuple

import torch

from . import lib as L


def _ptr(t):
    return 0 if t is None else (t if isinstance(t, int) else t.data_ptr())


def stream():
    return torch.cuda.current_stream().cuda_stream


def _chk(t, name):
    if t is None:
        return
    if not (t.is_cuda and t.dtype == torch.float32 and t.is_contiguous()):
        raise L.LdmkError(f"{name}: expected a contiguous float32 CUDA tensor, got {t.dtype} {t.device} "
                          f"contiguous={t.is_contiguous()}")

# ... 156 lines not shown
        e = h2_scale_exp(w)
        L.call("ldmk_pack_ps_h2", _ptr(w), N, K, 1, N, batch, K * N, e, 0, _ptr(out), stream())
        ptr = out.data_ptr()
        _WPS_H2_EXP[ptr] = (weakref.ref(out), e)
        weakref.finalize(out, _WPS_H2_EXP.pop, ptr, None)
    else:
        L.call("ldmk_pack_ps", _ptr(w), N, K, 1, N, batch, K * N, _ptr(out), stream())
    return out


def fold_pout(w2, b2, wpo, bpo, dtype=torch.float32):
    w2d, wpod = w2.double(), wpo.reshape(wpo.shape[0], wpo.shape[1]).double()
    w = torch.cat([w2d.t() @ wpod.t(), wpod.t()], 0)
    b = b2.double() @ wpod.t() + bpo.double()
    return w.to(dtype).contiguous(), b.to(dtype).contiguous()


FOLD_POUT_H2_MIN_RATIO = 2.0 ** -16


def fold_pout_h2_ok(w, k0):
    top, bot = float(w[:k0].abs().max().item()), float(w[k0:].abs().max().item())
    return min(top, bot) >= FOLD_POUT_H2_MIN_RATIO * max(top, bot) > 0.0


def ln_stats_ps(x2d, eps=1e-5, out=None, ps=None, guard=0.0, flag=None, h2_flag=None):
    rows, c = x2d.shape
    if out is None:
        out = torch.empty(rows, 2, device=x2d.device, dtype=torch.float32)
    if ps is None:
        ps = ps_empty(rows, c, 1, x2d.device, h2=h2_flag is not None)
    if h2_flag is not None:
        L.call("ldmk_ln_stats_ps_h2", _ptr(x2d), rows, c, float(eps), _ptr(out), _ptr(ps), float(guard), _ptr(flag), _ptr(h2_flag), stream())
    else:
        L.call("ldmk_ln_stats_ps", _ptr(x2d), rows, c, float(eps), _ptr(out), _ptr(ps), float(guard), _ptr(flag), stream())
    return out, ps


def unpack_ps_h2(ps, rows, k):
    nb = (rows + 31) // 32
    t = ps.reshape(-1).view(torch.float16).reshape(nb, k // 16, 2, 2, 32, 8)
    t = t.permute(2, 0, 4, 1, 3, 5).reshape(2, nb * 32, k)[:, :rows]
    return t[0].float(), t[1].float()


def unpack_ps(ps, rows, k):
    nb = (rows + 31) // 32
    t = ps.reshape(-1).view(torch.bfloat16).reshape(nb, k // 16, 3, 2, 32, 8)
    t = t.permute(2, 0, 4, 1, 3, 5).reshape(3, nb * 32, k)[:, :rows]
    return t[0].float(), t[1].float(), t[2].float()


def make_post_args(src, M, N, rows_per_sample, nslab=1, slab_stride=None, bias=None, batch_vec=None, batch_vec_ld=0,
                   residual=None, ldr=None, geglu=False, raw_out=None, ld_raw=None, norm=L.POST_NONE, x1=None, c1=0,
                   gamma=None, beta=None, eps=1e-5, silu=False, norm_out=None, ld_norm=None, groups=32, alpha=1.0):
    a = L.PostArgs()
    a.src, a.nslab, a.slab_stride = _ptr(src), nslab, (M * N if slab_stride is None else slab_stride)
    a.M, a.N, a.rows_per_sample, a.alpha = M, N, rows_per_sample, alpha
    a.bias, a.batch_vec, a.batch_vec_ld = _ptr(bias), _ptr(batch_vec), batch_vec_ld
    a.residual, a.ldr = _ptr(residual), (N if ldr is None else ldr)
    a.geglu = 1 if geglu else 0
    a.raw_out, a.ld_raw = _ptr(raw_out), ((N // 2 if geglu else N) if ld_raw is None else ld_raw)
    a.norm, a.x1, a.c1, a.groups, a.eps = norm, _ptr(x1), c1, groups, float(eps)
    a.gamma, a.beta, a.silu = _ptr(gamma), _ptr(beta), 1 if silu else 0
    a.norm_out, a.ld_norm = _ptr(norm_out), ((N + c1) if ld_norm is None else ld_norm)
    return a


def post(args, device=None):
    need = L.load().ldmk_post_scratch_elems(C.byref(args))
    if need > 0 and not args.gn_scratch:
        scratch = torch.empty(need, device=device if device is not None else torch.device("cuda", torch.cuda.current_device()),
                              dtype=torch.float32)
        args.gn_scratch, args.gn_scratch_elems = scratch.data_ptr(), need
        args._scratch = scratch
    L.call("ldmk_post", C.byref(args), stream())


def make_igemm_args(M, N, K, a0, c0, w, out, ldc, rows_per_sample, a1=None, c1=0, conv=None, tf=L.TF_NONE,
                    tf_coef=None, row_stats=None, ln_gamma=None, ln_beta=None, b_trans=False, ldb=None, bias=None,
                    batch_vec=None, batch_vec_ld=0, residual=None, epi=L.EPI_NONE, batch=1, a_bstride=0, w_bstride=0,
                    out_bstride=0, alpha=1.0, splitk=0, splitk_ws=None, w_frag=None, tile_cfg=0, compute=0, ln_colsum=None,
                    splitk_counters=None, raw_slabs=False, a_split=None, w_bf16t=None, a_ps=None, w_ps=None, out_ps=None,
                    range_flag=None, attn_kv=None, a_ps1=None, a_ps_k0=0):
    a = L.IgemmArgs()
    a._keep = (a0, a1, w, out, tf_coef, row_stats, ln_gamma, ln_beta, bias, batch_vec, residual, splitk_ws, w_frag, ln_colsum,
               splitk_counters, a_split, w_bf16t, a_ps, w_ps, out_ps)
    a.M, a.N, a.K = M, N, K
    a.a0, a.a1, a.c0, a.c1 = _ptr(a0), _ptr(a1), c0, c1
    if conv is not None:
        a.a_mode = L.A_CONV3X3
        a.in_h, a.in_w, a.out_h, a.out_w, a.stride, a.pad_lo, a.upsample = conv
    else:
        a.a_mode = L.A_ROWS
    a.a_tf = tf
    a.tf_coef, a.row_stats, a.ln_gamma, a.ln_beta = _ptr(tf_coef), _ptr(row_stats), _ptr(ln_gamma), _ptr(ln_beta)
    a.rows_per_sample = rows_per_sample
    a.w, a.b_trans = _ptr(w), 1 if b_trans else 0
    a.ldb = ldb if ldb is not None else (K if b_trans else N)
    a.bias, a.batch_vec, a.batch_vec_ld = _ptr(bias), _ptr(batch_vec), batch_vec_ld
    a.residual, a.epi = _ptr(residual), epi
    a.out, a.ldc, a.batch = _ptr(out), ldc, batch
    a.a_bstride, a.w_bstride, a.out_bstride = a_bstride, w_bstride, out_bstride
    a.alpha = alpha
    a.splitk = splitk
    a.w_frag, a.tile_cfg, a.compute = _ptr(w_frag), tile_cfg, compute
    a.ln_colsum = _ptr(ln_colsum)
    a.raw_slabs = 1 if raw_slabs else 0
    if splitk_counters is not None:
        a.splitk_counters, a.splitk_counters_len = splitk_counters.data_ptr(), splitk_counters.numel()
    if splitk_ws is not None:
        a.splitk_ws, a.splitk_ws_elems = splitk_ws.data_ptr(), splitk_ws.numel()
    if w_bf16t is not None:
        a.w_split, a.w_split_ld = _ptr(w_bf16t), w_bf16t.shape[-1]
    if a_split is not None:
        a.a_split, a.a_split_ld = _ptr(a_split), a_split.shape[-1]
    if a_ps is not None:
        a.a_ps, a.w_ps, a.out_ps = _ptr(a_ps), _ptr(w_ps), _ptr(out_ps)
        if a_ps1 is not None:
            a.a_ps1, a.a_ps_k0 = _ptr(a_ps1), int(a_ps_k0)
            a._keep = a._keep + (a_ps1,)
        if batch > 1:
            a.a_ps_bstride, a.w_ps_bstride = a_ps.shape[-1], w_ps.shape[-1]
        hit = _WPS_H2_EXP.get(w_ps.data_ptr())
        if hit is not None and hit[0]() is w_ps:
            a.compute, a.w_scale_exp, a.range_flag = L.COMPUTE_F16X2, hit[1], _ptr(range_flag)
            a._keep = a._keep + (range_flag,)
            if attn_kv is not None:
                a.attn_kv_out, a.attn_tokens, a.attn_heads = _ptr(attn_kv[0]), int(attn_kv[1]), int(attn_kv[2])
                a._keep = a._keep + (attn_kv[0],)
        else:
            a.compute = L.COMPUTE_BF16X3
        return a
    if compute == L.COMPUTE_BF16X3 and not set_split(a):
        raise ValueError("COMPUTE_BF16X3: no split images registered for this weight (ops.pack_wsplit) or b_trans set")
    if compute == L.COMPUTE_F16X2 and not set_split_h2(a, range_flag):
        raise ValueError("COMPUTE_F16X2: no fp16 images registered for this weight (ops.pack_wsplit_h2), b_trans set, or no range_flag")
    return a


def igemm(args):
    L.call("ldmk_igemm", C.byref(args), stream())


class WeightImage(NamedTuple):
    image: torch.Tensor
    ld: int
    bstride: int
    src: weakref.ref
    version: int
    scale_exp: int
    compute: int


_IMAGES = {}


def _pack_image(w, batch, compute):
    assert w.is_contiguous() and ((w.dim() == 3 and w.shape[0] == batch) if batch > 1 else w.dim() == 2)
    K, N = w.shape[-2:]
    ld = (K + 7) // 8 * 8
    if compute == L.COMPUTE_F16X2:
        e = h2_scale_exp(w)
        out = torch.empty(batch, 2, N, ld, device=w.device, dtype=torch.float16)
        L.call("ldmk_pack_wsplit_h2", _ptr(w), K, N, N, batch, K * N, e, _ptr(out), ld, stream())
    else:
        e, out = 0, torch.empty(batch, 3, N, ld, device=w.device, dtype=torch.bfloat16)
        L.call("ldmk_pack_wsplit", _ptr(w), K, N, N, batch, K * N, _ptr(out), ld, stream())
    key = (w.data_ptr(), compute)
    _IMAGES[key] = WeightImage(out, ld, out.shape[1] * N * ld, weakref.ref(w), w._version, e, compute)
    weakref.finalize(w, _drop_image, key, out.data_ptr())
    return out


def _drop_image(key, img_ptr):
    hit = _IMAGES.get(key)
    if hit is not None and hit.image.data_ptr() == img_ptr:
        del _IMAGES[key]


def image_of(w_ptr, compute):
    hit = _IMAGES.get((w_ptr, compute))
    if hit is None:
        return None
    src = hit.src()
    if src is None or src.data_ptr() != w_ptr or src._version != hit.version:
        del _IMAGES[(w_ptr, compute)]
        return None
    return hit


def attach_image(a, img, range_flag=None):
    a.w_split, a.w_split_ld, a.w_split_bstride = img.image.data_ptr(), img.ld, img.bstride
    if img.compute == L.COMPUTE_F16X2:
        a.w_scale_exp, a.range_flag = img.scale_exp, range_flag.data_ptr()
        a._keep = getattr(a, "_keep", ()) + (range_flag,)
    a.compute = img.compute


def pack_wsplit(w, batch=1):
    return _pack_image(w, batch, L.COMPUTE_BF16X3)


def pack_wsplit_h2(w, batch=1):
    return _pack_image(w, batch, L.COMPUTE_F16X2)


def pack_wbf16t(w):
    assert w.dim() == 2 and w.is_contiguous()
    K, N = w.shape
# ... 343 lines not shown
```

dsml_thesis_amd/switches.py:

```python
import os

SWITCHES = {
    "LDMK_SPLIT_BF16": ("1", "arithmetic", "0: every GEMM and the attention on the f32 matrix-core form (v_mfma_f32_32x32x2_f32); the "
                        "f32_mfma_form leg of bench.py", "tolerance"),
    "LDMK_F16X2": ("1", "arithmetic", "0: split products from the exact bf16x3 split (six bf16 MFMAs, operands bit-exact) instead of "
                   "F16X2 (three fp16 MFMAs, range-checked per site); the bf16x3_form leg of bench.py", "tolerance"),
    "LDMK_LN_UNFOLDED": (None, "arithmetic", "set: LayerNorm applied in the GEMM prologue instead of folded through the product (what "
                         "the folded-LayerNorm guard switches a model to by itself)", "tolerance"),
    "LDMK_LN_GUARD_RATIO": ("4.0", "arithmetic", "|mean| / std of a token row above which the folded LayerNorm raises its guard", None),
    "LDMK_ATTN_H2_MIN_TOKENS": ("512", "arithmetic", "self attention runs in F16X2 from this many tokens per sample, bf16x3 below", None),
    "LDMK_H2_CONV_RULE": ("1", "arithmetic", "0: untabled long-K convolutions (K >= 1440) do not take the F16X2 rule (they stay on the f32 matrix-core form of their plan: other bits, same tolerance)", "tolerance"),
    "LDMK_PS": ("1", "route", "0: no pre-split (PS layout, LDS-DMA) GEMM tiles: every GEMM back on the LDS-tiled plan of its shape (that plan's "
                "tile and K split), no conv-mode tile, no folded proj_out -- other bits, same tolerance (tile for tile, at equal split-K, "
                "a pre-split kernel gives the LDS-tiled kernel's bits: tests/test_ps_gpu.py)", "tolerance"),
    "LDMK_PSC": ("1", "route", "0: no conv-mode pre-split tile for 3x3 convolutions: the listed shapes return to their other route (Winograd for "
                 "the wide ones, the in-register split on that route's plan) -- other bits, same tolerance (at equal split-K the tile gives "
                 "the LDS-tiled F16X2 convolution's bits: tests/test_ps_conv_gpu.py)", "tolerance"),
    "LDMK_PSC_FORCE": (None, "route", "'cfg,splitk': force the conv-mode pre-split tile for every eligible convolution (A/B runs)", None),
    "LDMK_POUT_PS": ("0", "route", "1: SpatialTransformer.proj_out on a pre-split tile instead of the row GEMM (measured slower; another arithmetic: other bits, same tolerance)", "tolerance"),
    "LDMK_FOLD_POUT": ("1", "route", "0: the last block's ff.net.2 and proj_out stay two GEMMs instead of one pre-split GEMM on two A "
                       "sources with the composed weight (other bits, same tolerance)", "tolerance"),
    "LDMK_ATTN_PS": ("1", "route", "0: attn1.to_out does not read the attention result in the PS layout (its GEMM leaves the pre-split tile: other bits, same tolerance)", "tolerance"),
    "LDMK_ATTN_PRESPLIT": ("1", "route", "0: K / V are split inside the attention kernel instead of once by their producer; same bits", "bits"),
    "LDMK_ATTN_PRESPLIT_MIN_TOKENS": ("2048", "route", "tokens per sample from which K / V are pre-split", None),
    "LDMK_QKV_TILES": ("1", "route", "0: the fused QKV projection does not write the attention's K / V tiles from its epilogue (the attention's own pre-pass splits them; same bits)", "bits"),
    "LDMK_NO_WINOGRAD": (None, "route", "set: no Winograd F(2x2,3x3) convolutions and no phase-split upsampling convolutions (direct "
                         "implicit GEMM everywhere; other bits, same tolerance)", "tolerance"),
    "LDMK_WINO_MIN_TILES": ("256", "route", "Winograd from this many 2x2 output tiles at the plan-policy batch", None),
    "LDMK_WINO_MIN_CIN": ("320", "route", "Winograd / phase-split upsampling from this many input channels", None),
    "LDMK_NO_SMALL_ROUTE": (None, "route", "set: batch 1-2 jobs run the batched launch program instead of the small-batch route (other kernels: other bits, same tolerance)", "tolerance"),
    "LDMK_SMALL_ROWS": ("4096", "route", "rows (batch x pixels at the policy batch) up to which the small-batch route is taken", None),
    "LDMK_SPLITK_IN_LAUNCH": (None, "route", "set: split-K slabs combined by each tile's last workgroup instead of a reduce launch "
                              "(measured slower; the same output bits per GEMM, but its GroupNorm records are summed in another order: other bits, same tolerance)", "tolerance"),
    "LDMK_TRAIN_NO_PACKED_W": (None, "route", "set: the training step's bf16 GEMMs read fp32 weights instead of the packed bf16 copies (rounded to bf16 in the kernel as the packing does; same bits)", "bits"),
    "LDMK_ATTN_QT": (None, "route", "1 | 2: query tiles per wave of the staged f32 attention kernel (A/B hook; other bits, same tolerance)", "tolerance"),
    "LDMK_NO_PLAN_TABLE": (None, "plan", "set: ignore igemm_plans.json (the library's built-in tile heuristic plans every GEMM)", None),
    "LDMK_PLAN_MAX_RATIO": ("0", "plan", "> 0: a tuned plan is used only within this ratio of its tuned row count (0: nearest at any "
                            "distance)", None),
    "LDMK_PLAN_TABLE": (None, "plan", "a file that replaces the `f32` section of igemm_plans.json (a flat {key: [cfg, splitk]} file as "
                        "the tuning tools write it, or another merged file whose section is taken)", None),
    "LDMK_X3_TABLE": (None, "plan", "the same for the `bf16x3` section", None),
    "LDMK_H2_TABLE": (None, "plan", "the same for the `f16x2` section", None),
    "LDMK_PS_TABLE": (None, "plan", "the same for the `ps_bf16x3` section (pre-split tiles)", None),
    "LDMK_PS_H2_TABLE": (None, "plan", "the same for the `ps_f16x2` section (pre-split tiles, F16X2)", None),
    "LDMK_LIBRARY": (None, "runtime", "path of the libldmk.so to load instead of the in-tree one", None),
    "LDMK_FORCE_COLLECTIVE": (None, "runtime", "set: parallel.all_gather_items issues the real all-gather at world size 1 too (RCCL "
                              "rehearsal; bench.py sets it under LDMK_BENCH_FORCE_DIST)", None),
    "LDMK_LIB_OUT": (None, "build", "output path of the build (an A/B build next to the shipped library)", None),
    "LDMK_HIPCC_FLAGS": ("", "build", "extra hipcc flags, part of the build digest (-DLDMK_PS_PROBES, -DLDMK_IG_STAMPS: probe builds "
                         "for tools/; the shipped library carries neither)", None),
    "LDMK_ATTN_QB": (None, "library", "1 | 2: 32-query blocks per wave of the pre-split attention kernels (default by token count); "
                     "same bits -- but two blocks per wave at a multiple of 256 tokens bring the F16X2 kernel's pipelined loop with them: "
                     "the same bits under LDMK_ATTN_PIPE=1 | 0, other bits within the same tolerance under its default 2", "bits"),
    "LDMK_ATTN_XCD": ("1", "library", "0: F16X2 attention workgroups in launch order instead of re-dealt over the XCDs; same bits", "bits"),
    "LDMK_ATTN_PIPE": ("2", "library", "F16X2 attention key loop: 2 pipelined + lazy running maximum, 1 pipelined with the exact "
                       "maximum, 0 phase-separated (1 and 0: same bits)", "bits"),
    "LDMK_IG_NFAST": ("1", "library", "0: LDS-tiled igemm workgroups in row-major tile order instead of column tiles adjacent; same bits", "bits"),
    "LDMK_IG_LEAN": ("1", "library", "0: the general igemm epilogue everywhere instead of the operand-set specialised copies; same bits", "bits"),
    "LDMK_PS_NFAST": ("1", "library", "as LDMK_IG_NFAST, pre-split tiles; same bits", "bits"),
    "LDMK_PS_LEAN": ("1", "library", "as LDMK_IG_LEAN, pre-split tiles; same bits", "bits"),
    "LDMK_WINO_STAGED": ("1", "library", "0: the Winograd input / output transforms on their first kernels (a thread loads its own 4x4 "
                         "window / walks a band's tiles) instead of the LDS-staged / vectorised ones; same bits", "bits"),
    "LDMK_WGRAD_TR": ("1", "library", "0: bf16 weight-gradient GEMM with the strided gather instead of transposed LDS reads (A/B); dW the same bits, the fused "
                      "bias gradient's fp32 column sums in another order (other bits, same tolerance)", "tolerance"),
    "LDMK_BENCH_BACKEND": ("nccl", "bench", "'gloo': rehearse the N > 1 path of bench.py on a one-GPU box", None),
    "LDMK_BENCH_FORCE_DIST": (None, "bench", "set: create the process group and issue the clip leg's collective with a single rank", None),
}

PROBE_ONLY = ("LDMK_PS_DEBUG", "LDMK_PS_STAGGER")


def get(name, default=None):
    if name not in SWITCHES:
        raise KeyError(f"{name} is not a registered switch (dsml_thesis_amd/switches.py)")
    return os.environ.get(name, default)


def table_markdown():
    rows = ["| switch | default | scope | contract | effect |", "|---|---|---|---|---|"]
    for name, (default, scope, doc, contract) in SWITCHES.items():
        shown = "unset" if default is None else ("`" + (default or "''") + "`")
        rows.append(f"| `{name}` | {shown} | {scope} | {contract or '-'} | {doc} |")
    return "\n".join(rows)


if __name__ == "__main__":
    print(table_markdown())
```

dsml_thesis_amd/unet.py:

```python
import math
import os

import torch
import torch.nn as nn

from . import lib as L
from . import switches
from . import ops
from .engine import ArithSites, NetBuilder, Program, far_from_tuned, split_enabled as engine_split_enabled, ps_enabled as engine_ps_enabled, f16x2_enabled

LN_GUARD_RATIO = float(switches.get("LDMK_LN_GUARD_RATIO", "4.0"))


ATTN_PRESPLIT_MIN_TOKENS = int(switches.get("LDMK_ATTN_PRESPLIT_MIN_TOKENS", "2048"))
ATTN_H2_MIN_TOKENS = int(switches.get("LDMK_ATTN_H2_MIN_TOKENS", "512"))


def ln_unfolded_default():
    return bool(switches.get("LDMK_LN_UNFOLDED"))


class _Params(nn.Module):
    def __init__(self, **shapes):
        super().__init__()
        for name, shape in shapes.items():
            self.register_parameter(name, nn.Parameter(torch.empty(*shape), requires_grad=False))


class _Slots(nn.Module):

    def __init__(self, **children):
        super().__init__()
        for k, m in children.items():
            self.add_module(k.lstrip("_"), m)


def _conv_params(cin, cout, k):
    return _Params(weight=(cout, cin, k, k), bias=(cout,))


def _lin_params(cin, cout, bias=True):
    return _Params(weight=(cout, cin), bias=(cout,)) if bias else _Params(weight=(cout, cin))


def _norm_params(c):
    return _Params(weight=(c,), bias=(c,))


def _res_block(cin, cout, emb_ch, scale_shift=False, updown=None):
    ch = dict(in_layers=_Slots(_0=_norm_params(cin), _2=_conv_params(cin, cout, 3)),
              emb_layers=_Slots(_1=_lin_params(emb_ch, 2 * cout if scale_shift else cout)),
              out_layers=_Slots(_0=_norm_params(cout), _3=_conv_params(cout, cout, 3)))
    if cin != cout:
        ch["skip_connection"] = _conv_params(cin, cout, 1)
    m = _Slots(**ch)
    m.kind, m.cin, m.cout, m.scale_shift, m.updown = "res", cin, cout, bool(scale_shift), updown
    return m


def _attn(dim, ctx_dim):
    return _Slots(to_q=_lin_params(dim, dim, False), to_k=_lin_params(ctx_dim, dim, False),
                  to_v=_lin_params(ctx_dim, dim, False), to_out=_Slots(_0=_lin_params(dim, dim)))


def _spatial_transformer(ch, heads, d_head, depth, context_dim):
    inner = heads * d_head
    blocks = nn.ModuleList()
    for _ in range(depth):
        blocks.append(_Slots(
            attn1=_attn(inner, inner),
            ff=_Slots(net=_Slots(_0=_Slots(proj=_lin_params(inner, inner * 8)), _2=_lin_params(inner * 4, inner))),
            attn2=_attn(inner, context_dim if context_dim is not None else inner),
            norm1=_norm_params(inner), norm2=_norm_params(inner), norm3=_norm_params(inner)))
    m = _Slots(norm=_norm_params(ch), proj_in=_conv_params(ch, inner, 1), transformer_blocks=blocks,
               proj_out=_conv_params(inner, ch, 1))
    m.kind, m.ch, m.heads, m.d_head, m.depth = "st", ch, heads, d_head, depth
    return m


def _attention_block(ch, heads, new_order=False):
    m = _Slots(norm=_norm_params(ch), qkv=_Params(weight=(3 * ch, ch, 1), bias=(3 * ch,)),
               proj_out=_Params(weight=(ch, ch, 1), bias=(ch,)))
    m.kind, m.ch, m.heads, m.d_head, m.new_order = "attn", ch, heads, ch // heads, bool(new_order)
    return m


def _seq(*mods):
    s = nn.Module()
    for i, m in enumerate(mods):
        s.add_module(str(i), m)
    s.layers = list(mods)
    return s


def pack_spatial_transformer(P, sd, prefix, m):
    P[prefix + "pin"] = ops.pack_linear(sd[prefix + "proj_in.weight"])
    P[prefix + "pout"] = ops.pack_linear(sd[prefix + "proj_out.weight"])
    for d in range(m.depth):
# ... 79 lines not shown
        bq = sd[prefix + "qkv.bias"].reshape(heads, 3, d).permute(1, 0, 2).reshape(3 * ch).contiguous()
    P[prefix + "aqkv"] = ops.pack_linear(w)
    P[prefix + "aqkv#b"] = bq
    P[prefix + "apout"] = ops.pack_linear(sd[prefix + "proj_out.weight"].reshape(ch, ch).contiguous())


def emit_attention_block(nb_, P, sd, prefix, m, x, h, w):
    pg, n = nb_.pg, nb_.n
    p_ = lambda t: 0 if t is None else t.data_ptr()
    hw = h * w
    rows = n * hw
    xr = x.reshape(rows, m.ch)
    coef = nb_.gn(x, None, hw, sd[prefix + "norm.weight"], sd[prefix + "norm.bias"], 1e-5)
    with nb_.site(prefix + "attn"):
        qkv = nb_.lin(xr, P[prefix + "aqkv"], P[prefix + "aqkv#b"], hw, tf=L.TF_AFFINE, tf_coef=coef, wf=P.get(prefix + "aqkv#f"))
        nb_.release(coef)
        att = pg.alloc(rows, m.ch)
        emit_self_attention(nb_, qkv, att, hw, m.heads, m.d_head)
        nb_.release(qkv)
    with nb_.site(prefix + "proj_out"):
        out = nb_.lin(att, P[prefix + "apout"], sd[prefix + "proj_out.bias"], hw, residual=xr, stats=True, wf=P.get(prefix + "apout#f"))
    nb_.release(att)
    return out.view(n, h, w, m.ch)


def pack_gemm_copies(P, unfolded=False):
    for k in [k for k in P if k.rsplit(".", 1)[-1] in ("pin", "pout", "qkv_ln", "o1", "q2_ln", "o2", "ff1_ln", "ff2", "skip",
                                                        "c1", "c2", "aqkv", "apout")
              or (unfolded and k.rsplit(".", 1)[-1] in ("qkv", "ff1", "q2"))]:
        wf = ops.pack_wfrag(P[k])
        if wf is not None:
            P[k + "#f"] = wf
    if engine_split_enabled():
        for k in list(P):
            tail = k.rsplit(".", 1)[-1]
            if tail in ("pin", "pout", "qkv_ln", "o1", "ff1_ln", "ff2", "skip", "c1", "c2", "w", "aqkv", "apout") or (unfolded and tail in ("qkv", "ff1")):
                if P[k].dim() == 2:
                    P[k + "#s"] = ops.pack_wsplit(P[k])
                    if f16x2_enabled():
                        P[k + "#h"] = ops.pack_wsplit_h2(P[k])
            elif tail in ("c1#wg", "c2#wg", "w#up"):
                P[k + "#s"] = ops.pack_wsplit(P[k], batch=P[k].shape[0])
                if f16x2_enabled():
                    P[k + "#h"] = ops.pack_wsplit_h2(P[k], batch=P[k].shape[0])
    if engine_ps_enabled():
        for k in list(P):
            tail = k.rsplit(".", 1)[-1]
            if tail in ("qkv_ln", "ff1_ln", "ff2", "o1", "pout", "ffpo") and P[k].dim() == 2 and P[k].shape[0] % 32 == 0 and P[k].shape[1] % 32 == 0:
                P[k + "#p"] = ops.pack_wps(P[k])
            elif tail in ("c1#wg", "c2#wg", "w#up") and P[k].shape[1] % 32 == 0 and P[k].shape[2] % 32 == 0:
                P[k + "#p"] = ops.pack_wps(P[k], batch=P[k].shape[0])
        if f16x2_enabled():
            for k in list(P):
                tail = k.rsplit(".", 1)[-1]
                if tail in ("qkv_ln", "ff1_ln", "ff2", "o1", "pout") and P[k].dim() == 2 and P[k].shape[0] % 32 == 0 and P[k].shape[1] % 32 == 0:
                    P[k + "#p2"] = ops.pack_wps(P[k], h2=True)
                elif tail == "ffpo" and ops.fold_pout_h2_ok(P[k], P[k].shape[0] - P[k].shape[0] // 5):
                    P[k + "#p2"] = ops.pack_wps(P[k], h2=True)
                elif tail in ("c1#wg", "c2#wg", "w#up") and P[k].shape[1] % 32 == 0 and P[k].shape[2] % 32 == 0:
                    P[k + "#p2"] = ops.pack_wps(P[k], batch=P[k].shape[0], h2=True)
                elif tail in ("c1", "c2") and P[k].dim() == 2 and P[k].shape[0] % (9 * 32) == 0 and P[k].shape[1] % 32 == 0:
                    P[k + "#pc2"] = ops.pack_wps(P[k], h2=True)


def emit_spatial_transformer(nb_, ctx_pg, P, sd, prefix, m, x, h, w, L_ctx, ctx_in, context_dim, unfolded=False, ln_flag=None):
    pg, n = nb_.pg, nb_.n
    gn, lin = nb_.gn, nb_.lin
    p_ = lambda t: 0 if t is None else t.data_ptr()
    hw = h * w
    C_ = m.heads * m.d_head
    rows = n * hw
    xr = x.reshape(rows, m.ch)
    coef = gn(x, None, hw, sd[prefix + "norm.weight"], sd[prefix + "norm.bias"], 1e-6)
    with nb_.site(prefix + "proj_in"):
        hcur = lin(xr, P[prefix + "pin"], sd[prefix + "proj_in.bias"], hw, tf=L.TF_AFFINE, tf_coef=coef, wf=P.get(prefix + "pin#f"))
    nb_.release(coef)
    stats = pg.alloc(rows, 2)

    hf = lambda: nb_.h2_flag
    psfx = lambda: "#p2" if hf() is not None else "#p"

    kv_state = {"tiles": None}

    def ln_lin(x2d, wkey, geglu, out_ps=None, attn_kv=None, keep_xs=False):
        wp = P[wkey]
        N_ = wp.shape[1]
        h2_flag = hf()
        plan = nb_.ps_query(rows, N_, C_, tf=L.TF_LAYERNORM_FOLDED, epi=L.EPI_GEGLU if geglu else L.EPI_NONE) if wkey + psfx() in P else None
        if plan is not None:
            xs = pg.alloc_ps(rows, C_)
            if h2_flag is not None:
                pg.add("ldmk_ln_stats_ps_h2", p_(x2d), rows, C_, 1e-5, p_(stats), p_(xs), LN_GUARD_RATIO, p_(ln_flag), p_(h2_flag))
            else:
                pg.add("ldmk_ln_stats_ps", p_(x2d), rows, C_, 1e-5, p_(stats), p_(xs), LN_GUARD_RATIO, p_(ln_flag))
            kw = {}
            if attn_kv is not None and h2_flag is not None and int(plan[0]) in (23, 27) and int(plan[1]) <= 1:
                kw["attn_kv"] = attn_kv
                kv_state["tiles"] = attn_kv[0]
            y = nb_.lin_ps(plan, rows, C_, xs, wp, P[wkey + psfx()], P[wkey + "#b"], hw, geglu=geglu, out_ps=out_ps,
                           tf=L.TF_LAYERNORM_FOLDED, row_stats=stats, ln_colsum=P[wkey + "#cs"], **kw)
            if keep_xs:
                return xs
            nb_.release(xs)
            return y
        assert out_ps is None
        pg.add("ldmk_ln_stats_guard", p_(x2d), rows, C_, 1e-5, p_(stats), LN_GUARD_RATIO, p_(ln_flag))
        return lin(x2d, wp, P[wkey + "#b"], hw, geglu=geglu, tf=L.TF_LAYERNORM_FOLDED, row_stats=stats,
                   ln_colsum=P[wkey + "#cs"], wf=P.get(wkey + "#f"))

    hc_ps = plan_p = None
    ff_site = None

    def attn1_section(q, hcur):
        h2_flag = hf()
        if unfolded:
            pg.add("ldmk_ln_stats", p_(hcur), rows, C_, 1e-5, p_(stats))
            qkv = lin(hcur, P[q + "qkv"], None, hw, tf=L.TF_LAYERNORM, row_stats=stats,
                      ln_gamma=sd[q + "norm1.weight"], ln_beta=sd[q + "norm1.bias"], wf=P.get(q + "qkv#f"))
        else:
            kv_state["tiles"] = None
            kvt = None
            if (h2_flag is not None and hw >= ATTN_H2_MIN_TOKENS and hw % 64 == 0 and m.d_head == 32
                    and switches.get("LDMK_QKV_TILES", "1") != "0"):
                kvt = pg.alloc(pg.lib.ldmk_attn_kv_split_h2_bytes(n, hw, m.heads), dtype=torch.uint8)
            qkv = ln_lin(hcur, q + "qkv_ln", False, attn_kv=None if kvt is None else (kvt, hw, m.heads))
            if kvt is not None and kv_state["tiles"] is None:
                nb_.release(kvt)
                kvt = None
        plan_o = (nb_.ps_query(rows, C_, C_) if (q + "o1" + psfx() in P and L_ctx == 1 and hw % 32 == 0 and switches.get("LDMK_ATTN_PS", "1") != "0"
                                                 and m.d_head == 32
                                                 and (hw >= ATTN_H2_MIN_TOKENS if h2_flag is not None else attention_presplit(hw))) else None)
        att = None if plan_o is not None else pg.alloc(rows, C_)
        att_ps = pg.alloc_ps(rows, C_) if plan_o is not None else None
        kv_tiles = None if unfolded else kv_state["tiles"]
        emit_self_attention(nb_, qkv, att, hw, m.heads, m.d_head, att_ps=att_ps, kv_tiles=kv_tiles)
        nb_.release(qkv)
        if kv_tiles is not None:
            nb_.release(kv_tiles)
        if L_ctx != 1:
            return lin(att, P[q + "o1"], sd[q + "attn1.to_out.0.bias"], hw, residual=hcur, out=hcur, wf=P.get(q + "o1#f")), att
        v = ctx_pg.alloc(n, C_)
        ctx_pg.add("ldmk_dense_small", p_(ctx_in), context_dim, p_(P[q + "v2"]), 0, p_(v), C_, n,
                   context_dim, C_, 0)
        cvec = ctx_pg.alloc(n, C_)
        ctx_pg.add("ldmk_dense_small", p_(v), C_, p_(P[q + "o2"]), p_(sd[q + "attn2.to_out.0.bias"]), p_(cvec),
                   C_, n, C_, C_, 0)
        if plan_o is not None:
            h1 = nb_.lin_ps(plan_o, rows, C_, att_ps, P[q + "o1"], P[q + "o1" + psfx()], sd[q + "attn1.to_out.0.bias"], hw, out=hcur,
                            residual=hcur, batch_vec=cvec, batch_vec_ld=C_)
            nb_.release(att_ps)
        else:
            h1 = lin(att, P[q + "o1"], sd[q + "attn1.to_out.0.bias"], hw, residual=hcur, out=hcur,
                     batch_vec=cvec, batch_vec_ld=C_, wf=P.get(q + "o1#f"))
            nb_.release(att)
        return h1, None

    def attn2_section(q, h1, att):
        kk = ctx_pg.alloc(n * L_ctx, C_)
        vv = ctx_pg.alloc(n * L_ctx, C_)
        ctx_pg.add("ldmk_dense_small", p_(ctx_in), context_dim, p_(P[q + "k2"]), 0, p_(kk), C_,
                   n * L_ctx, context_dim, C_, 0)
        ctx_pg.add("ldmk_dense_small", p_(ctx_in), context_dim, p_(P[q + "v2"]), 0, p_(vv), C_,
                   n * L_ctx, context_dim, C_, 0)
        if unfolded:
            pg.add("ldmk_ln_stats", p_(h1), rows, C_, 1e-5, p_(stats))
            q2 = lin(h1, P[q + "q2"], None, hw, tf=L.TF_LAYERNORM, row_stats=stats, ln_gamma=sd[q + "norm2.weight"],
                     ln_beta=sd[q + "norm2.bias"], out=att, wf=P.get(q + "q2#f"))
        else:
            pg.add("ldmk_ln_stats_guard", p_(h1), rows, C_, 1e-5, p_(stats), LN_GUARD_RATIO, p_(ln_flag))
            q2 = lin(h1, P[q + "q2_ln"], P[q + "q2_ln#b"], hw, tf=L.TF_LAYERNORM_FOLDED, row_stats=stats,
                     ln_colsum=P[q + "q2_ln#cs"], out=att, wf=P.get(q + "q2_ln#f"))
        a2 = pg.alloc(rows, C_)
        if m.d_head == 32:
            pg.add("ldmk_attn_cross", p_(q2), C_, p_(kk), p_(vv), C_, p_(a2), C_, n, hw, L_ctx, m.heads, m.d_head ** -0.5)
        elif m.d_head in (40, 64, 80):
            pg.add("ldmk_attn_cross_d", p_(q2), C_, p_(kk), p_(vv), C_, p_(a2), C_, n, hw, L_ctx, m.heads, m.d_head, m.d_head ** -0.5)
        else:
            raise NotImplementedError(f"cross attention over a context of {L_ctx} tokens with heads of width {m.d_head} (built: 32, 40, 64, 80)")
        h2 = lin(a2, P[q + "o2"], sd[q + "attn2.to_out.0.bias"], hw, residual=h1, out=h1, wf=P.get(q + "o2#f"))
        nb_.release(att, a2)
        return h2

    def ff_section(q, h2, last):
        Nf = P[q + "ff2"].shape[0]
        plan_g = plan_f = None
        if not unfolded and q + "ff1_ln" + psfx() in P and q + "ff2" + psfx() in P:
            plan_g = nb_.ps_query(rows, 2 * Nf, C_, tf=L.TF_LAYERNORM_FOLDED, epi=L.EPI_GEGLU)
            plan_f = nb_.ps_query(rows, C_, Nf)
        if plan_g is not None and plan_f is not None:
            f_ps = pg.alloc_ps(rows, Nf)
            plan_fp = (nb_.ps_query(rows, m.ch, Nf + C_) if (last and prefix + "ffpo" + psfx() in P
                                                            and switches.get("LDMK_FOLD_POUT", "1") != "0") else None)
            if plan_fp is not None:
                xs = ln_lin(h2, q + "ff1_ln", True, out_ps=f_ps, keep_xs=True)
                out = nb_.lin_ps(plan_fp, rows, Nf + C_, f_ps, P[prefix + "ffpo"], P[prefix + "ffpo" + psfx()], P[prefix + "ffpo#b"], hw,
                                 residual=xr, stats=True, a_ps1=xs, a_ps_k0=Nf)
                nb_.release(f_ps, xs, h2)
                return None, None, None, out
            ln_lin(h2, q + "ff1_ln", True, out_ps=f_ps)
            plan_p = (nb_.ps_query(rows, m.ch, C_) if (last and prefix + "pout" + psfx() in P and plan_f[1] <= 1
                                                       and switches.get("LDMK_POUT_PS", "0") == "1") else None)
            hc_ps = pg.alloc_ps(rows, C_) if plan_p is not None else None
            hcur = nb_.lin_ps(plan_f, rows, Nf, f_ps, P[q + "ff2"], P[q + "ff2" + psfx()], sd[q + "ff.net.2.bias"], hw, out=h2, residual=h2,
                              out_ps=hc_ps)
            nb_.release(f_ps)
            return hcur, hc_ps, plan_p, None
        if unfolded:
            pg.add("ldmk_ln_stats", p_(h2), rows, C_, 1e-5, p_(stats))
            f = lin(h2, P[q + "ff1"], P[q + "ff1b"], hw, geglu=True, tf=L.TF_LAYERNORM, row_stats=stats,
                    ln_gamma=sd[q + "norm3.weight"], ln_beta=sd[q + "norm3.bias"], wf=P.get(q + "ff1#f"))
        else:
            f = ln_lin(h2, q + "ff1_ln", True)
        hcur = lin(f, P[q + "ff2"], sd[q + "ff.net.2.bias"], hw, residual=h2, out=h2, wf=P.get(q + "ff2#f"))
        nb_.release(f)
        return hcur, None, None, None

    for d in range(m.depth):
        q = f"{prefix}transformer_blocks.{d}."
        with nb_.site(q + "attn1"):
            h1, att = attn1_section(q, hcur)
        if L_ctx == 1:
            h2 = h1
        else:
            with nb_.site(q + "attn2"):
                h2 = attn2_section(q, h1, att)
        ff_site = q + "ff"
        with nb_.site(ff_site):
            hcur, hc_ps, plan_p, out = ff_section(q, h2, d == m.depth - 1)
    if out is not None:
        nb_.release(stats)
        return out.view(n, h, w, m.ch)
    if hc_ps is not None:
        with nb_.site(ff_site):
            out = nb_.lin_ps(plan_p, rows, C_, hc_ps, P[prefix + "pout"], P[prefix + "pout" + psfx()], sd[prefix + "proj_out.bias"], hw, residual=xr,
                             stats=True)
        nb_.release(hc_ps)
    else:
        with nb_.site(prefix + "proj_out"):
            out = lin(hcur, P[prefix + "pout"], sd[prefix + "proj_out.bias"], hw, residual=xr, stats=True, wf=P.get(prefix + "pout#f"))
    nb_.release(hcur, stats)
    return out.view(n, h, w, m.ch)


MAX_ARITHMETIC_PASSES = 5


def rerun_if_flags_tripped(unet_of):
    import functools

    def deco(fn):
        @functools.wraps(fn)
        def wrapped(self, *args, **kwargs):
            if torch.cuda.is_current_stream_capturing():
                return fn(self, *args, **kwargs)
            unet = unet_of(self)
            rng = torch.cuda.get_rng_state()
            for _ in range(MAX_ARITHMETIC_PASSES):
                out = fn(self, *args, **kwargs)
                if not unet.flags_tripped():
                    break
                torch.cuda.set_rng_state(rng)
            return out
        return wrapped
    return deco


rerun_if_layernorm_guard_tripped = rerun_if_flags_tripped


class UNetModel(nn.Module):
    def __init__(self, image_size, in_channels, model_channels, out_channels, num_res_blocks,
                 attention_resolutions, dropout=0, channel_mult=(1, 2, 4, 8), conv_resample=True, dims=2,
                 num_classes=None, use_checkpoint=False, use_fp16=False, num_heads=-1, num_head_channels=-1,
                 num_heads_upsample=-1, use_scale_shift_norm=False, resblock_updown=False,
                 use_new_attention_order=False, use_spatial_transformer=False, transformer_depth=1,
                 context_dim=None, n_embed=None, legacy=True):
        super().__init__()
        if dims != 2:
            raise NotImplementedError("UNetModel: only dims=2")
        if n_embed is not None:
            raise NotImplementedError("UNetModel: n_embed (the id-predictor head) is not part of the sampling path built here")
        if use_new_attention_order and use_spatial_transformer:
            pass
        if not conv_resample:
            raise NotImplementedError("UNetModel: conv_resample=False")
        if use_fp16:
            raise NotImplementedError("UNetModel: fp32 only (reference precision)")
        if dropout != 0 and self.training:
            pass
        if use_spatial_transformer:
            assert context_dim is not None, "use_spatial_transformer needs context_dim (openaimodel.py:471-472)"
        else:
            assert context_dim is None, "context_dim needs use_spatial_transformer (openaimodel.py:474-475)"
        self.use_spatial_transformer = bool(use_spatial_transformer)
        if isinstance(context_dim, (list, tuple)) or type(context_dim).__name__ == "ListConfig":
            context_dim = list(context_dim)
            assert len(context_dim) == 1, "a single context dim is supported"
            context_dim = context_dim[0]
        if num_heads == -1:
            assert num_head_channels != -1, "Either num_heads or num_head_channels has to be set"
        if num_heads_upsample == -1:
            num_heads_upsample = num_heads
        attention_resolutions = list(attention_resolutions)
        channel_mult = list(channel_mult)
        self.image_size, self.in_channels, self.model_channels = image_size, in_channels, model_channels
        self.out_channels, self.num_res_blocks = out_channels, num_res_blocks
        self.attention_resolutions, self.channel_mult = attention_resolutions, channel_mult
        self.dropout, self.conv_resample, self.num_classes = dropout, conv_resample, num_classes
        self.use_checkpoint, self.dtype = use_checkpoint, torch.float32
        self.num_heads, self.num_head_channels, self.num_heads_upsample = num_heads, num_head_channels, num_heads_upsample
        self.context_dim, self.transformer_depth = context_dim, transformer_depth
# ... 471 lines not shown
```

include/ldmk.h:

```cpp
#ifndef LDMK_H
#define LDMK_H
#ifdef __cplusplus
extern "C" {
#endif

#define LDMK_OK 0
#define LDMK_EINVAL (-1)
#define LDMK_EHIP (-2)
#define LDMK_ENOMEM (-3)

int ldmk_version(void);
const char* ldmk_last_error(void);
int ldmk_init(int device);

int ldmk_switch_value(const char* name);
int ldmk_switch_override(const char* name, int value);

enum { LDMK_A_ROWS = 0, LDMK_A_CONV3X3 = 1 };
enum { LDMK_TF_NONE = 0, LDMK_TF_AFFINE = 1, LDMK_TF_AFFINE_SILU = 2, LDMK_TF_LAYERNORM = 3,
       LDMK_TF_LAYERNORM_FOLDED = 4 };
enum { LDMK_EPI_NONE = 0, LDMK_EPI_GEGLU = 1 };
enum { LDMK_COMPUTE_F32 = 0, LDMK_COMPUTE_BF16 = 1, LDMK_COMPUTE_BF16X3 = 2, LDMK_COMPUTE_F16X2 = 3 };
#define LDMK_F16X2_A_EXP 6
#define LDMK_F16X2_RANGE 1000.0f

typedef struct ldmk_igemm_args {
  int M, N, K;
  const float* a0;
  const float* a1;
  int c0, c1;
  int a_mode;
  int in_h, in_w;
  int out_h, out_w;
  int stride, pad_lo;
  int upsample;
  int a_tf;
  const float* tf_coef;
  const float* row_stats;
  const float* ln_gamma;
  const float* ln_beta;
  int rows_per_sample;
  const float* w;
  int b_trans, ldb;
  const float* bias;
  const float* batch_vec;
  int batch_vec_ld;
  const float* residual;
  int epi;
  float* out;
  int ldc;
  int batch;
  long long a_bstride, w_bstride, out_bstride;
  float alpha;
  int tile_cfg;
  int splitk;
  float* splitk_ws;
  long long splitk_ws_elems;
  float* stats_out;
  int compute;
  int* splitk_counters;
  int splitk_counters_len;
  const float* w_frag;
  const float* ln_colsum;
  int raw_slabs;
  const float* skip_a0;
  const float* skip_a1;
  int skip_c0, skip_c1;
  const void* w_split;
  int w_split_ld;
  long long w_split_bstride;
  const void* a_split;
  int a_split_ld;
  const void* a_ps;
  long long a_ps_bstride;
  const void* w_ps;
  long long w_ps_bstride;
  void* out_ps;
  int w_scale_exp;
  int* range_flag;
  void* attn_kv_out;
  int attn_tokens;
  int attn_heads;
  const void* a_ps1;
  int a_ps_k0;
} ldmk_igemm_args;

long long ldmk_ps_bytes(int rows, int k);
int ldmk_pack_ps(const float* src, int rows, int k, long long row_stride, long long k_stride, int batch, long long src_bstride,
                 void* dst, void* stream);
int ldmk_ln_stats_ps(const float* x, int rows, int c, float eps, float* stats, void* dst, float guard, int* flag, void* stream);

long long ldmk_ps_bytes_h2(int rows, int k);
int ldmk_pack_ps_h2(const float* src, int rows, int k, long long row_stride, long long k_stride, int batch, long long src_bstride,
                    int scale_exp, int* range_flag, void* dst, void* stream);
int ldmk_ln_stats_ps_h2(const float* x, int rows, int c, float eps, float* stats, void* dst, float guard, int* flag, int* range_flag,
                        void* stream);
int ldmk_gn_apply_ps_h2(const float* x0, int c0, const float* x1, int c1, const float* coef, void* y_ps, int n, int hw, int silu,
                        int* range_flag, void* stream);

int ldmk_pack_wsplit(const float* w, int K, int N, int ldb, int batch, long long w_bstride, void* out, int ld_out, void* stream);
int ldmk_pack_wsplit_h2(const float* w, int K, int N, int ldb, int batch, long long w_bstride, int scale_exp, void* out, int ld_out,
                        void* stream);
int ldmk_pack_wbf16t(const float* w, int K, int N, int ldb, void* out, int ld_out, void* stream);

int ldmk_igemm(const ldmk_igemm_args* args, void* stream);
long long ldmk_igemm_workspace_elems(const ldmk_igemm_args* args);
int ldmk_igemm_check(const ldmk_igemm_args* args);
long long ldmk_wfrag_elems(int K, int N);
int ldmk_pack_wfrag(const float* w, int ldb, int K, int N, float* wfrag, void* stream);
int ldmk_fold_layernorm(const float* w, int ldb, int K, int N, const float* gamma, const float* beta, const float* bias,
                        float* w_out, float* colsum, float* bias_out, void* stream);
int ldmk_igemm_plan(const ldmk_igemm_args* args, int* tile_cfg, int* splitk);

long long ldmk_winograd_tiles(int n, int h, int w);
int ldmk_winograd_input(const float* x0, int c0, const float* x1, int c1, const float* coef, int silu, int n, int h, int w,
                        float* v, void* stream);
int ldmk_winograd_input_ps(const float* x0, int c0, const float* x1, int c1, const float* coef, int silu, int n, int h, int w,
                           void* v_ps, void* stream);
int ldmk_winograd_input_ps_h2(const float* x0, int c0, const float* x1, int c1, const float* coef, int silu, int n, int h, int w,
                              void* v_ps, int* range_flag, void* stream);
int ldmk_winograd_output(const float* m, const float* bias, const float* batch_vec, int batch_vec_ld, const float* residual,
                         float* out, float* stats_out, int n, int h, int w, int cout, void* stream);
int ldmk_winograd_input_ps_route(int n, int h, int w, int c0, int c1);
int ldmk_winograd_output_route(int n, int h, int w, int cout, int with_stats);
int ldmk_winograd_input_ps_v1(const float* x0, int c0, const float* x1, int c1, const float* coef, int silu, int n, int h, int w,
                              void* v_ps, void* stream);
int ldmk_winograd_input_ps_h2_v1(const float* x0, int c0, const float* x1, int c1, const float* coef, int silu, int n, int h, int w,
                                 void* v_ps, int* range_flag, void* stream);
int ldmk_winograd_output_v1(const float* m, const float* bias, const float* batch_vec, int batch_vec_ld, const float* residual,
                            float* out, float* stats_out, int n, int h, int w, int cout, void* stream);

int ldmk_upconv_gather(const float* x, int c, int n, int h, int w, float* a, void* stream);
int ldmk_upconv_gather_ps(const float* x, int c, int n, int h, int w, void* a_ps, void* stream);
int ldmk_upconv_gather_ps_h2(const float* x, int c, int n, int h, int w, void* a_ps, int* range_flag, void* stream);
int ldmk_upconv_scatter(const float* planes, const float* bias, float* out, float* stats_out, int n, int h, int w, int cout,
                        void* stream);

int ldmk_gn_chunks(int hw);
int ldmk_gn_partial(const float* x, int c, int n, int hw, float* partial, void* stream);
int ldmk_gn_finalize(const float* partial0, int c0, const float* partial1, int c1, int n, int hw, int groups,
                     float eps, const float* gamma, const float* beta, float* coef, void* stream);
int ldmk_gn_coef(const float* x0, int c0, const float* x1, int c1, int n, int hw, int groups, float eps,
                 const float* gamma, const float* beta, float* partial, float* coef, void* stream);
int ldmk_ln_stats(const float* x, int rows, int c, float eps, float* stats, void* stream);
int ldmk_ln_stats_guard(const float* x, int rows, int c, float eps, float* stats, float guard, int* flag, void* stream);
int ldmk_ln_stats_split(const float* x, int rows, int C, float eps, float* stats, void* split, int ld_split, void* stream);
int ldmk_gn_apply(const float* x0, int c0, const float* x1, int c1, const float* coef, float* y, int n, int hw,
                  int silu, void* stream);
int ldmk_resample2(const float* x, float* y, int n, int h, int w, int c, int up, void* stream);
int ldmk_gn_coef_film(float* coef, const float* emb, int ld, int n, int c, void* stream);

enum { LDMK_POST_NONE = 0, LDMK_POST_GROUPNORM = 1, LDMK_POST_LAYERNORM = 2 };
typedef struct ldmk_post_args {
  const float* src;
  int nslab;
  long long slab_stride;
  int M, N;
  int rows_per_sample;
  float alpha;
  const float* bias;
  const float* batch_vec;
  int batch_vec_ld;
  const float* residual;
  int ldr;
  int geglu;
  float* raw_out;
  int ld_raw;
// ... 206 lines not shown
```

Before: 1190 sample-steps/s.

## Fuse LN3 statistics into attn1.to_out epilogue via per-span row moments

The attn1.to_out pre-split GEMM epilogue now writes its output in the PS layout and also emits per-160-column (mean, M2) moments for each row. The following GEGLU projection then combines these moments into mean/rstd inline, in place of the separate LayerNorm statistics-and-pack pass. This removes one full read/write pass over the hidden state and one kernel launch per transformer block. In exchange the epilogue does extra reductions, the fp32 output write can be skipped in some routes, and the summation order changes, so results differ slightly in the last bits.

```diff
diff --git a/dsml_thesis_amd/csrc/igemm.hip b/dsml_thesis_amd/csrc/igemm.hip
--- a/dsml_thesis_amd/csrc/igemm.hip
+++ b/dsml_thesis_amd/csrc/igemm.hip
@@ -1272,6 +1272,8 @@
                "ldmk_igemm: compute=%d", a.compute);
   const bool ps_tile = a.tile_cfg > kNumCfg + kNumRCfg + kNumSCfg + kNumWCfg;
   LDMK_REQUIRE(!a.a_ps1 || (ps_tile && a.a_ps), "ldmk_igemm: a_ps1 (second A source) is read by the pre-split tiles only, next to a_ps");
+  LDMK_REQUIRE((!a.row_moments_out && !a.row_moment_spans && !a.out_ps_range_flag) || (ps_tile && a.a_ps),
+               "ldmk_igemm: row_moments_out / row_moment_spans / out_ps_range_flag belong to the pre-split tiles (tile_cfg 23..28 / 31..33)");
   if (a.compute == LDMK_COMPUTE_BF16X3 && !ps_tile) {
     LDMK_REQUIRE(a.w_split && !a.b_trans && a.w_split_ld >= a.K && a.w_split_ld % 8 == 0,
                  "ldmk_igemm: LDMK_COMPUTE_BF16X3 needs w_split (ldmk_pack_wsplit), b_trans = 0, w_split_ld >= K and a multiple of 8");
diff --git a/dsml_thesis_amd/csrc/igemm_ps.hip b/dsml_thesis_amd/csrc/igemm_ps.hip
--- a/dsml_thesis_amd/csrc/igemm_ps.hip
+++ b/dsml_thesis_amd/csrc/igemm_ps.hip
@@ -49,7 +49,37 @@
 __device__ __attribute__((aligned(16))) const float kPsZeros[4] = {0.f, 0.f, 0.f, 0.f};
 
 constexpr int PS_KV_TILE = 16 * 1024;
-template <int TM, int TN, bool TR, int PL = 3, bool KV = false, int LEAN = 0>
+__device__ __forceinline__ float ps_half_sum(float x) {
+  const auto r = __builtin_amdgcn_permlane32_swap(__float_as_uint(x), __float_as_uint(x), false, false);
+  return __uint_as_float(r[0]) + __uint_as_float(r[1]);
+}
+constexpr int PS_SPAN = 160;
+
+__device__ __forceinline__ void ps_ln_from_moments(const ldmk_igemm_args& p, const int r, float& mean, float& rstd, bool& guard_up) {
+  const int spans = p.row_moment_spans;
+  const float2* __restrict__ mp = reinterpret_cast<const float2*>(p.row_stats) + (long long)r * spans;
+  float2 m[4];
+#pragma unroll
+  for (int j = 0; j < 4; ++j) m[j] = mp[j < spans ? j : spans - 1];
+  float ms = m[0].x, q = m[0].y;
+#pragma unroll
+  for (int j = 1; j < 4; ++j) {
+    ms += j < spans ? m[j].x : 0.f;
+    q += j < spans ? m[j].y : 0.f;
+  }
+  mean = ms * (1.0f / (float)spans);
+  float dd = 0.f;
+#pragma unroll
+  for (int j = 0; j < 4; ++j) {
+    const float d = j < spans ? m[j].x - mean : 0.f;
+    dd = fmaf(d, d, dd);
+  }
+  q = fmaf((float)PS_SPAN, dd, q);
+  rstd = 1.0f / sqrtf(q / (float)p.K + p.ln_eps);
+  guard_up |= !(fabsf(mean) * rstd <= p.ln_guard);
+}
+
+template <int TM, int TN, bool TR, int PL = 3, bool KV = false, int LEAN = 0, bool MOM = false, bool MIN = false>
 __device__ __forceinline__ void ps_epilogue(const ldmk_igemm_args& p, f32x16 (&acc)[TM][TN], const int rowbase, const int colbase,
                                             const int splitk, const int ks, const int bz, float* __restrict__ ws, const int lane,
                                             float* __restrict__ kv_ts = nullptr) {
@@ -86,6 +116,7 @@
     const float* __restrict__ bip = p.bias ? p.bias : kPsZeros;
     const float* __restrict__ rsp = p.residual ? p.residual + (long long)bz * p.out_bstride : kPsZeros;
     const unsigned mcs = lnf ? ~0u : 0u, mbi = p.bias ? ~0u : 0u, mrs = p.residual ? ~0u : 0u, mbv = p.batch_vec ? ~0u : 0u;
+    bool guard_up = false;
     bool bad_ps = false;
 #pragma unroll
     for (int i = 0; i < TM; ++i) {
@@ -93,7 +124,15 @@
       const bool rok = L_ANY || row < p.M;
       const int rr = rok ? row : p.M - 1;
       float mean = 0.f, rstd = 1.f;
-      if (lnf) { const float2 st = stats2[rr]; mean = st.x; rstd = st.y; }
+      if (lnf) {
+        if constexpr (MIN) {
+          ps_ln_from_moments(p, rr, mean, rstd, guard_up);
+        } else {
+          if (p.row_moment_spans > 0) ps_ln_from_moments(p, rr, mean, rstd, guard_up);
+          else { const float2 st = stats2[rr]; mean = st.x; rstd = st.y; }
+        }
+      }
+      float msum[4] = {0.f, 0.f, 0.f, 0.f};
       const float* __restrict__ bvp = p.batch_vec ? p.batch_vec + (long long)(rr / p.rows_per_sample) * p.batch_vec_ld : kPsZeros;
       const unsigned rowoff = (unsigned)rr * (unsigned)p.ldc;
       const long long psrow = ((long long)((rowbase + 32 * i) >> 5) * Kbo) * (PL * 1024) + l31 * 16 + half * 8;
@@ -175,6 +214,10 @@
               v.x += bv[q].x; v.y += bv[q].y; v.z += bv[q].z; v.w += bv[q].w;
               v.x += rs[q].x; v.y += rs[q].y; v.z += rs[q].z; v.w += rs[q].w;
             }
+            if constexpr (MOM) {
+              acc[i][jt][4 * q] = v.x; acc[i][jt][4 * q + 1] = v.y; acc[i][jt][4 * q + 2] = v.z; acc[i][jt][4 * q + 3] = v.w;
+              msum[q] += (v.x + v.y) + (v.z + v.w);
+            }
             if constexpr (KV) {
               if (kv_tile) { kvv[4 * q] = v.x; kvv[4 * q + 1] = v.y; kvv[4 * q + 2] = v.z; kvv[4 * q + 3] = v.w; }
             }
@@ -260,8 +303,21 @@
           }
         }
       }
-    }
-    if (bad_ps) *p.range_flag = 1;
+      if constexpr (MOM) {
+        static_assert(32 * TN == PS_SPAN && !KV, "row moments: one 160-column span per wave tile");
+        const float mean_j = ps_half_sum((msum[0] + msum[1]) + (msum[2] + msum[3])) / (float)PS_SPAN;
+        float q4[4] = {0.f, 0.f, 0.f, 0.f};
+#pragma unroll
+        for (int j = 0; j < TN; ++j)
+#pragma unroll
+          for (int r = 0; r < 16; ++r) { const float d = acc[i][j][r] - mean_j; q4[r & 3] = fmaf(d, d, q4[r & 3]); }
+        const float m2 = ps_half_sum((q4[0] + q4[1]) + (q4[2] + q4[3]));
+        if (rok && half == 0 && colbase < p.N)
+          reinterpret_cast<float2*>(p.row_moments_out)[(long long)row * (p.N / PS_SPAN) + colbase / PS_SPAN] = make_float2(mean_j, m2);
+      }
+    }
+    if (bad_ps) *(p.out_ps_range_flag ? p.out_ps_range_flag : p.range_flag) = 1;
+    if (guard_up && p.ln_guard_flag) *p.ln_guard_flag = 1;
     return;
   } else {
     if (splitk > 1) {
@@ -290,7 +346,7 @@
   }
 }
 
-template <int NWM, int NWN, int TM, int TN, int NS, bool TR, int PL = 3, bool KV = false>
+template <int NWM, int NWN, int TM, int TN, int NS, bool TR, int PL = 3, bool KV = false, bool MOMK = false>
 __global__ __launch_bounds__(64 * NWM * NWN, 2) void igemm_ps_kernel(const ldmk_igemm_args p, const int splitk, float* __restrict__ ws, const int dbg_arg, const int nfast) {
   const int dbg = PS_PROBES ? dbg_arg : 0;
   constexpr int NW = NWM * NWN;
@@ -445,7 +501,19 @@
       ps_epilogue<TM, TN, TR, PL, true>(p, acc, m0 + wm * 32 * TM, n0 + wn * 32 * TN, splitk, ks, bz, ws, lane,
                                          reinterpret_cast<float*>(smem_ps) + wave * (32 * 33));
   } else {
-    if (lean == 1) ps_epilogue<TM, TN, TR, PL, false, 1>(p, acc, m0 + wm * 32 * TM, n0 + wn * 32 * TN, splitk, ks, bz, ws, lane);
+    if constexpr (MOMK) {
+      static_assert(TR && 32 * TN == PS_SPAN && !KV, "row moments: transposed epilogue, 160 columns per wave");
+      if (lean == 2) ps_epilogue<TM, TN, TR, PL, false, 2, true>(p, acc, m0 + wm * 32 * TM, n0 + wn * 32 * TN, splitk, ks, bz, ws, lane);
+      else if (lean == 4) ps_epilogue<TM, TN, TR, PL, false, 4, true>(p, acc, m0 + wm * 32 * TM, n0 + wn * 32 * TN, splitk, ks, bz, ws, lane);
+      else ps_epilogue<TM, TN, TR, PL, false, 0, true>(p, acc, m0 + wm * 32 * TM, n0 + wn * 32 * TN, splitk, ks, bz, ws, lane);
+      return;
+    }
+    if (lean == 1) {
+      if (TR && p.row_moment_spans > 0)
+        ps_epilogue<TM, TN, TR, PL, false, 1, false, TR>(p, acc, m0 + wm * 32 * TM, n0 + wn * 32 * TN, splitk, ks, bz, ws, lane);
+      else
+        ps_epilogue<TM, TN, TR, PL, false, 1>(p, acc, m0 + wm * 32 * TM, n0 + wn * 32 * TN, splitk, ks, bz, ws, lane);
+    }
     else if (lean == 2) ps_epilogue<TM, TN, TR, PL, false, 2>(p, acc, m0 + wm * 32 * TM, n0 + wn * 32 * TN, splitk, ks, bz, ws, lane);
     else if (lean == 3) ps_epilogue<TM, TN, TR, PL, false, 3>(p, acc, m0 + wm * 32 * TM, n0 + wn * 32 * TN, splitk, ks, bz, ws, lane);
     else if (lean == 4) ps_epilogue<TM, TN, TR, PL, false, 4>(p, acc, m0 + wm * 32 * TM, n0 + wn * 32 * TN, splitk, ks, bz, ws, lane);
@@ -732,14 +800,14 @@
                                {256, 160, false}, {256, 128, true},
                                {256, 160, false}, {256, 128, true}, {128, 256, true}};
 
-template <int NWM, int NWN, int TM, int TN, int NS, bool TR, int PL = 3, bool KV = false>
+template <int NWM, int NWN, int TM, int TN, int NS, bool TR, int PL = 3, bool KV = false, bool MOMK = false>
 static int ps_launch(const ldmk_igemm_args& a, int splitk, float* ws, hipStream_t st) {
   constexpr int BM = 32 * TM * NWM, BN = 32 * TN * NWN;
   constexpr size_t lds = (size_t)NS * (BM / 32 + BN / 32) * PL * 1024;
   static_assert(lds <= 160 * 1024, "LDS ring exceeds 160 KiB");
   static bool attr = false;
   if (!attr) {
-    (void)hipFuncSetAttribute(reinterpret_cast<const void*>(igemm_ps_kernel<NWM, NWN, TM, TN, NS, TR, PL, KV>),
+    (void)hipFuncSetAttribute(reinterpret_cast<const void*>(igemm_ps_kernel<NWM, NWN, TM, TN, NS, TR, PL, KV, MOMK>),
                               hipFuncAttributeMaxDynamicSharedMemorySize, (int)lds);
     attr = true;
   }
@@ -749,7 +817,7 @@
   const int nfast_env = switch_value(SW_PS_NFAST);
   const int lean_env = switch_value(SW_PS_LEAN);
   const int nfast = (nfast_env && (a.N + BN - 1) / BN > 1 && (a.M + BM - 1) / BM >= 8 ? 1 : 0) | (lean_env ? 0 : 2);
-  hipLaunchKernelGGL((igemm_ps_kernel<NWM, NWN, TM, TN, NS, TR, PL, KV>), dim3(tiles, splitk, a.batch > 1 ? a.batch : 1), dim3(64 * NWM * NWN), lds,
+  hipLaunchKernelGGL((igemm_ps_kernel<NWM, NWN, TM, TN, NS, TR, PL, KV, MOMK>), dim3(tiles, splitk, a.batch > 1 ? a.batch : 1), dim3(64 * NWM * NWN), lds,
                      st, a, splitk, ws, dbg, nfast);
   if (splitk > 1 && !a.raw_slabs) return launch_splitk_reduce(a, splitk, ws, st);
   return check_launch("ldmk_igemm(ps)");
@@ -996,6 +1064,23 @@
     return "no output";
   }
   if (a.stats_out && !a.out) return "stats_out needs out";
+  if (a.out_ps_range_flag && !a.out_ps) return "out_ps_range_flag is the flag of the out_ps check: it needs out_ps";
+  if (a.row_moments_out) {
+    if (a.a_mode != LDMK_A_ROWS || splitk > 1 || a.batch > 1 || a.stats_out) return "row_moments_out: rows mode, no split-K, no batching, no GroupNorm records (transposed epilogue)";
+    if (a.N % 160) return "row_moments_out: N must be a multiple of 160 (one (mean, M2) pair per 160-column span)";
+    if (pcfg != 0 && pcfg != 1 && pcfg != 3 && pcfg != 4 && pcfg != 8) return "row_moments_out: a tile whose waves own 160 columns (tile_cfg 23, 24, 26, 27, 31)";
+    if (a.a_tf != LDMK_TF_NONE || a.epi != LDMK_EPI_NONE || a.attn_kv_out) return "row_moments_out: no folded LayerNorm, no GEGLU, no fused QKV tiles";
+  }
+  if (a.row_moment_spans) {
+    if (a.a_tf != LDMK_TF_LAYERNORM_FOLDED) return "row_moment_spans: the moments stand in for (mean, rstd): a_tf must be LDMK_TF_LAYERNORM_FOLDED";
+    if (splitk > 1 || a.stats_out) return "row_moment_spans: no split-K (transposed epilogue)";
+    if ((a.row_moment_spans != 1 && a.row_moment_spans != 2 && a.row_moment_spans != 4) || a.K != 160 * a.row_moment_spans)
+      return "row_moment_spans: 1, 2 or 4 spans of 160 columns that make up K";
+    if (!(a.ln_eps > 0.f)) return "row_moment_spans: ln_eps must be positive";
+    if (a.ln_guard_flag && !(a.ln_guard > 0.f)) return "row_moment_spans: ln_guard must be positive";
+  } else if (a.ln_guard_flag) {
+    return "ln_guard_flag belongs to row_moment_spans (the statistics pass raises the guard otherwise)";
+  }
   if (a.attn_kv_out) {
     if (pl != 2 || (pcfg != 0 && pcfg != 4)) return "attn_kv_out: the F16X2 arithmetic on tile_cfg 23 / 27";
     if (a.stats_out || splitk > 1 || a.batch > 1 || a.epi != LDMK_EPI_NONE || a.out_ps || !a.out || !a.range_flag)
@@ -1014,6 +1099,24 @@
       case 1: return tr ? psc_launch<4, 2, 2, 5, true>(a, splitk, ws, st) : psc_launch<4, 2, 2, 5, false>(a, splitk, ws, st);
       case 3: return tr ? psc_launch<4, 2, 1, 5, true>(a, splitk, ws, st) : psc_launch<4, 2, 1, 5, false>(a, splitk, ws, st);
       default: return tr ? psc_launch<4, 1, 1, 5, true>(a, splitk, ws, st) : psc_launch<4, 1, 1, 5, false>(a, splitk, ws, st);
+    }
+  }
+  if (a.row_moments_out) {
+    if (a.compute == LDMK_COMPUTE_F16X2) {
+      switch (pcfg) {
+        case 0: return ps_launch<8, 1, 1, 5, 3, true, 2, false, true>(a, splitk, ws, st);
+        case 1: return ps_launch<4, 2, 2, 5, 3, true, 2, false, true>(a, splitk, ws, st);
+        case 3: return ps_launch<4, 2, 1, 5, 3, true, 2, false, true>(a, splitk, ws, st);
+        case 4: return ps_launch<4, 1, 1, 5, 3, true, 2, false, true>(a, splitk, ws, st);
+        default: return ps_launch<4, 1, 2, 5, 3, true, 2, false, true>(a, splitk, ws, st);
+      }
+    }
+    switch (pcfg) {
+      case 0: return ps_launch<8, 1, 1, 5, 3, true, 3, false, true>(a, splitk, ws, st);
+      case 1: return ps_launch<4, 2, 2, 5, 2, true, 3, false, true>(a, splitk, ws, st);
+      case 3: return ps_launch<4, 2, 1, 5, 3, true, 3, false, true>(a, splitk, ws, st);
+      case 4: return ps_launch<4, 1, 1, 5, 2, true, 3, false, true>(a, splitk, ws, st);
+      default: return ps_launch<4, 1, 2, 5, 2, true, 3, false, true>(a, splitk, ws, st);
     }
   }
   if (a.compute == LDMK_COMPUTE_F16X2 && a.attn_kv_out)
diff --git a/dsml_thesis_amd/lib.py b/dsml_thesis_amd/lib.py
--- a/dsml_thesis_amd/lib.py
+++ b/dsml_thesis_amd/lib.py
@@ -41,6 +41,8 @@
         ("w_scale_exp", C.c_int), ("range_flag", _fp),
         ("attn_kv_out", _fp), ("attn_tokens", C.c_int), ("attn_heads", C.c_int),
         ("a_ps1", _fp), ("a_ps_k0", C.c_int),
+        ("ln_eps", C.c_float), ("row_moments_out", _fp), ("out_ps_range_flag", _fp), ("ln_guard_flag", _fp),
+        ("row_moment_spans", C.c_int), ("ln_guard", C.c_float),
     ]
 
 
diff --git a/dsml_thesis_amd/ops.py b/dsml_thesis_amd/ops.py
--- a/dsml_thesis_amd/ops.py
+++ b/dsml_thesis_amd/ops.py
@@ -262,7 +262,8 @@
                     batch_vec=None, batch_vec_ld=0, residual=None, epi=L.EPI_NONE, batch=1, a_bstride=0, w_bstride=0,
                     out_bstride=0, alpha=1.0, splitk=0, splitk_ws=None, w_frag=None, tile_cfg=0, compute=0, ln_colsum=None,
                     splitk_counters=None, raw_slabs=False, a_split=None, w_bf16t=None, a_ps=None, w_ps=None, out_ps=None,
-                    range_flag=None, attn_kv=None, a_ps1=None, a_ps_k0=0):
+                    range_flag=None, attn_kv=None, a_ps1=None, a_ps_k0=0, row_moments_out=None, out_ps_range_flag=None,
+                    row_moments=None, ln_eps=1e-5, ln_guard=0.0, ln_guard_flag=None):
     a = L.IgemmArgs()
     a._keep = (a0, a1, w, out, tf_coef, row_stats, ln_gamma, ln_beta, bias, batch_vec, residual, splitk_ws, w_frag, ln_colsum,
                splitk_counters, a_split, w_bf16t, a_ps, w_ps, out_ps)
@@ -300,12 +301,23 @@
         if a_ps1 is not None:
             a.a_ps1, a.a_ps_k0 = _ptr(a_ps1), int(a_ps_k0)
             a._keep = a._keep + (a_ps1,)
+        if row_moments_out is not None:
+            a.row_moments_out = _ptr(row_moments_out)
+            a._keep = a._keep + (row_moments_out,)
+        if row_moments is not None:
+            assert row_stats is None
+            a.row_stats, a.row_moment_spans, a.ln_eps = _ptr(row_moments), K // 160, ln_eps
+            a.ln_guard, a.ln_guard_flag = ln_guard, _ptr(ln_guard_flag)
+            a._keep = a._keep + (row_moments, ln_guard_flag)
         if batch > 1:
             a.a_ps_bstride, a.w_ps_bstride = a_ps.shape[-1], w_ps.shape[-1]
         hit = _WPS_H2_EXP.get(w_ps.data_ptr())
         if hit is not None and hit[0]() is w_ps:
             a.compute, a.w_scale_exp, a.range_flag = L.COMPUTE_F16X2, hit[1], _ptr(range_flag)
             a._keep = a._keep + (range_flag,)
+            if out_ps_range_flag is not None:
+                a.out_ps_range_flag = _ptr(out_ps_range_flag)
+                a._keep = a._keep + (out_ps_range_flag,)
             if attn_kv is not None:
                 a.attn_kv_out, a.attn_tokens, a.attn_heads = _ptr(attn_kv[0]), int(attn_kv[1]), int(attn_kv[2])
                 a._keep = a._keep + (attn_kv[0],)
diff --git a/dsml_thesis_amd/switches.py b/dsml_thesis_amd/switches.py
--- a/dsml_thesis_amd/switches.py
+++ b/dsml_thesis_amd/switches.py
@@ -21,6 +21,9 @@
     "LDMK_FOLD_POUT": ("1", "route", "0: the last block's ff.net.2 and proj_out stay two GEMMs instead of one pre-split GEMM on two A "
                        "sources with the composed weight (other bits, same tolerance)", "tolerance"),
     "LDMK_ATTN_PS": ("1", "route", "0: attn1.to_out does not read the attention result in the PS layout (its GEMM leaves the pre-split tile: other bits, same tolerance)", "tolerance"),
+    "LDMK_LN3_EPI": ("1", "route", "0: the LN3 statistics pass stays between attn1.to_out and the GEGLU projection where both run on pre-split "
+                     "tiles, instead of to_out's epilogue writing the rows in the PS layout with their span moments (the statistics are "
+                     "summed in another order: other bits, same tolerance; both arms run in tests/test_ln3_epilogue_gpu.py)", None),
     "LDMK_ATTN_PRESPLIT": ("1", "route", "0: K / V are split inside the attention kernel instead of once by their producer; same bits", "bits"),
     "LDMK_ATTN_PRESPLIT_MIN_TOKENS": ("2048", "route", "tokens per sample from which K / V are pre-split", None),
     "LDMK_QKV_TILES": ("1", "route", "0: the fused QKV projection does not write the attention's K / V tiles from its epilogue (the attention's own pre-pass splits them; same bits)", "bits"),
diff --git a/dsml_thesis_amd/unet.py b/dsml_thesis_amd/unet.py
--- a/dsml_thesis_amd/unet.py
+++ b/dsml_thesis_amd/unet.py
@@ -14,6 +14,7 @@
 
 ATTN_PRESPLIT_MIN_TOKENS = int(switches.get("LDMK_ATTN_PRESPLIT_MIN_TOKENS", "2048"))
 ATTN_H2_MIN_TOKENS = int(switches.get("LDMK_ATTN_H2_MIN_TOKENS", "512"))
+LN3_EPI_TILES = (23, 24, 26, 27, 31)
 
 
 def ln_unfolded_default():
@@ -259,26 +260,31 @@
 
     kv_state = {"tiles": None}
 
-    def ln_lin(x2d, wkey, geglu, out_ps=None, attn_kv=None, keep_xs=False):
+    def ln_lin(x2d, wkey, geglu, out_ps=None, attn_kv=None, keep_xs=False, pre=None):
         wp = P[wkey]
         N_ = wp.shape[1]
         h2_flag = hf()
         plan = nb_.ps_query(rows, N_, C_, tf=L.TF_LAYERNORM_FOLDED, epi=L.EPI_GEGLU if geglu else L.EPI_NONE) if wkey + psfx() in P else None
+        assert pre is None or plan is not None
         if plan is not None:
-            xs = pg.alloc_ps(rows, C_)
-            if h2_flag is not None:
-                pg.add("ldmk_ln_stats_ps_h2", p_(x2d), rows, C_, 1e-5, p_(stats), p_(xs), LN_GUARD_RATIO, p_(ln_flag), p_(h2_flag))
+            if pre is not None:
+                xs, mom = pre
+                kw = dict(row_moments=mom, ln_eps=1e-5, ln_guard=LN_GUARD_RATIO, ln_guard_flag=ln_flag)
             else:
-                pg.add("ldmk_ln_stats_ps", p_(x2d), rows, C_, 1e-5, p_(stats), p_(xs), LN_GUARD_RATIO, p_(ln_flag))
-            kw = {}
+                xs = pg.alloc_ps(rows, C_)
+                if h2_flag is not None:
+                    pg.add("ldmk_ln_stats_ps_h2", p_(x2d), rows, C_, 1e-5, p_(stats), p_(xs), LN_GUARD_RATIO, p_(ln_flag), p_(h2_flag))
+                else:
+                    pg.add("ldmk_ln_stats_ps", p_(x2d), rows, C_, 1e-5, p_(stats), p_(xs), LN_GUARD_RATIO, p_(ln_flag))
+                kw = dict(row_stats=stats)
             if attn_kv is not None and h2_flag is not None and int(plan[0]) in (23, 27) and int(plan[1]) <= 1:
                 kw["attn_kv"] = attn_kv
                 kv_state["tiles"] = attn_kv[0]
             y = nb_.lin_ps(plan, rows, C_, xs, wp, P[wkey + psfx()], P[wkey + "#b"], hw, geglu=geglu, out_ps=out_ps,
-                           tf=L.TF_LAYERNORM_FOLDED, row_stats=stats, ln_colsum=P[wkey + "#cs"], **kw)
+                           tf=L.TF_LAYERNORM_FOLDED, ln_colsum=P[wkey + "#cs"], **kw)
             if keep_xs:
                 return xs
-            nb_.release(xs)
+            nb_.release(xs, None if pre is None else pre[1])
             return y
         assert out_ps is None
         pg.add("ldmk_ln_stats_guard", p_(x2d), rows, C_, 1e-5, p_(stats), LN_GUARD_RATIO, p_(ln_flag))
@@ -288,7 +294,17 @@
     hc_ps = plan_p = None
     ff_site = None
 
-    def attn1_section(q, hcur):
+    def ff_plans(q, last):
+        Nf = P[q + "ff2"].shape[0]
+        plan_g = plan_f = plan_fp = None
+        if not unfolded and q + "ff1_ln" + psfx() in P and q + "ff2" + psfx() in P:
+            plan_g = nb_.ps_query(rows, 2 * Nf, C_, tf=L.TF_LAYERNORM_FOLDED, epi=L.EPI_GEGLU)
+            plan_f = nb_.ps_query(rows, C_, Nf)
+        if plan_g is not None and plan_f is not None and last and prefix + "ffpo" + psfx() in P and switches.get("LDMK_FOLD_POUT", "1") != "0":
+            plan_fp = nb_.ps_query(rows, m.ch, Nf + C_)
+        return plan_g, plan_f, plan_fp
+
+    def attn1_section(q, hcur, ln3=None):
         h2_flag = hf()
         if unfolded:
             pg.add("ldmk_ln_stats", p_(hcur), rows, C_, 1e-5, p_(stats))
@@ -315,22 +331,29 @@
         if kv_tiles is not None:
             nb_.release(kv_tiles)
         if L_ctx != 1:
-            return lin(att, P[q + "o1"], sd[q + "attn1.to_out.0.bias"], hw, residual=hcur, out=hcur, wf=P.get(q + "o1#f")), att
+            return lin(att, P[q + "o1"], sd[q + "attn1.to_out.0.bias"], hw, residual=hcur, out=hcur, wf=P.get(q + "o1#f")), att, None
         v = ctx_pg.alloc(n, C_)
         ctx_pg.add("ldmk_dense_small", p_(ctx_in), context_dim, p_(P[q + "v2"]), 0, p_(v), C_, n,
                    context_dim, C_, 0)
         cvec = ctx_pg.alloc(n, C_)
         ctx_pg.add("ldmk_dense_small", p_(v), C_, p_(P[q + "o2"]), p_(sd[q + "attn2.to_out.0.bias"]), p_(cvec),
                    C_, n, C_, C_, 0)
+        pre = None
         if plan_o is not None:
-            h1 = nb_.lin_ps(plan_o, rows, C_, att_ps, P[q + "o1"], P[q + "o1" + psfx()], sd[q + "attn1.to_out.0.bias"], hw, out=hcur,
-                            residual=hcur, batch_vec=cvec, batch_vec_ld=C_)
+            kw, h1_fp32 = {}, True
+            if ln3 is not None and (h2_flag is None) == (ln3[0] is None) and int(plan_o[0]) in LN3_EPI_TILES and int(plan_o[1]) <= 1:
+                pre = (pg.alloc_ps(rows, C_), pg.alloc(rows, C_ // 160, 2))
+                kw = dict(out_ps=pre[0], row_moments_out=pre[1], out_ps_range_flag=ln3[0])
+                h1_fp32 = ln3[1]
+            nb_.lin_ps(plan_o, rows, C_, att_ps, P[q + "o1"], P[q + "o1" + psfx()], sd[q + "attn1.to_out.0.bias"], hw,
+                       out=hcur if h1_fp32 else None, residual=hcur, batch_vec=cvec, batch_vec_ld=C_, **kw)
+            h1 = hcur
             nb_.release(att_ps)
         else:
             h1 = lin(att, P[q + "o1"], sd[q + "attn1.to_out.0.bias"], hw, residual=hcur, out=hcur,
                      batch_vec=cvec, batch_vec_ld=C_, wf=P.get(q + "o1#f"))
             nb_.release(att)
-        return h1, None
+        return h1, None, pre
 
     def attn2_section(q, h1, att):
         kk = ctx_pg.alloc(n * L_ctx, C_)
@@ -358,23 +381,19 @@
         nb_.release(att, a2)
         return h2
 
-    def ff_section(q, h2, last):
+    def ff_section(q, h2, last, pre=None):
         Nf = P[q + "ff2"].shape[0]
-        plan_g = plan_f = None
-        if not unfolded and q + "ff1_ln" + psfx() in P and q + "ff2" + psfx() in P:
-            plan_g = nb_.ps_query(rows, 2 * Nf, C_, tf=L.TF_LAYERNORM_FOLDED, epi=L.EPI_GEGLU)
-            plan_f = nb_.ps_query(rows, C_, Nf)
+        plan_g, plan_f, plan_fp = ff_plans(q, last)
+        assert pre is None or (plan_g is not None and plan_f is not None)
         if plan_g is not None and plan_f is not None:
             f_ps = pg.alloc_ps(rows, Nf)
-            plan_fp = (nb_.ps_query(rows, m.ch, Nf + C_) if (last and prefix + "ffpo" + psfx() in P
-                                                            and switches.get("LDMK_FOLD_POUT", "1") != "0") else None)
             if plan_fp is not None:
-                xs = ln_lin(h2, q + "ff1_ln", True, out_ps=f_ps, keep_xs=True)
+                xs = ln_lin(h2, q + "ff1_ln", True, out_ps=f_ps, keep_xs=True, pre=pre)
                 out = nb_.lin_ps(plan_fp, rows, Nf + C_, f_ps, P[prefix + "ffpo"], P[prefix + "ffpo" + psfx()], P[prefix + "ffpo#b"], hw,
                                  residual=xr, stats=True, a_ps1=xs, a_ps_k0=Nf)
-                nb_.release(f_ps, xs, h2)
+                nb_.release(f_ps, xs, h2, None if pre is None else pre[1])
                 return None, None, None, out
-            ln_lin(h2, q + "ff1_ln", True, out_ps=f_ps)
+            ln_lin(h2, q + "ff1_ln", True, out_ps=f_ps, pre=pre)
             plan_p = (nb_.ps_query(rows, m.ch, C_) if (last and prefix + "pout" + psfx() in P and plan_f[1] <= 1
                                                        and switches.get("LDMK_POUT_PS", "0") == "1") else None)
             hc_ps = pg.alloc_ps(rows, C_) if plan_p is not None else None
@@ -394,8 +413,15 @@
 
     for d in range(m.depth):
         q = f"{prefix}transformer_blocks.{d}."
+        last = d == m.depth - 1
+        ln3 = None
+        if (not unfolded and L_ctx == 1 and C_ // 160 in (1, 2, 4) and C_ % 160 == 0 and switches.get("LDMK_LN3_EPI", "1") != "0"):
+            with nb_.site(q + "ff"):
+                plan_g, plan_f, plan_fp = ff_plans(q, last)
+                if plan_g is not None and plan_f is not None:
+                    ln3 = (hf(), plan_fp is None)
         with nb_.site(q + "attn1"):
-            h1, att = attn1_section(q, hcur)
+            h1, att, pre = attn1_section(q, hcur, ln3)
         if L_ctx == 1:
             h2 = h1
         else:
@@ -403,7 +429,7 @@
                 h2 = attn2_section(q, h1, att)
         ff_site = q + "ff"
         with nb_.site(ff_site):
-            hcur, hc_ps, plan_p, out = ff_section(q, h2, d == m.depth - 1)
+            hcur, hc_ps, plan_p, out = ff_section(q, h2, last, pre)
     if out is not None:
         nb_.release(stats)
         return out.view(n, h, w, m.ch)
diff --git a/include/ldmk.h b/include/ldmk.h
--- a/include/ldmk.h
+++ b/include/ldmk.h
@@ -83,6 +83,12 @@
   int attn_heads;
   const void* a_ps1;
   int a_ps_k0;
+  float ln_eps;
+  float* row_moments_out;
+  int* out_ps_range_flag;
+  int* ln_guard_flag;
+  int row_moment_spans;
+  float ln_guard;
 } ldmk_igemm_args;
 
 long long ldmk_ps_bytes(int rows, int k);
```

Result: no change. 1198 sample-steps/s, median of 6 (+0.7%).
